# jujuC31/NeutFEM

Measured on AMD Instinct MI355X. Metric: outer power-iters/sec (IAEA-3D RT0-P0 k-eigenvalue solve), higher is better.
Workload: dtype f64; 1 GPU; IAEA-3D resampled 256x256x256 RT0-P0 2g, full Schur path, CG tol 0.0001, Chebyshev; cells=16777216, groups=2, parallelism=1 process(es) x 1 z-slab(s) each; RCCL: interface planes + scalar all-reduces

## Files before the change

neutfem_amd/csrc/neutfem_hip.hip:

```cpp
#include "../../include/neutfem_hip.h"
#include "nf_kernels.h"
#include "nf_assembly.h"
#include "nf_line_groups.h"
#include "nf_small_eig.h"

#include <dlfcn.h>
#include <unistd.h>

#include <algorithm>
#include <chrono>
#include <climits>
#include <cmath>
#include <cstdarg>
#include <cstdint>
#include <cstdio>
#include <cstdlib>
#include <cstring>
#include <map>
#include <mutex>
#include <string>
#include <type_traits>
#include <utility>
#include <vector>

// ... 42 lines not shown
};
static Rccl g_rccl;
static bool trace_comm() { static int on = -1; if (on < 0) { const char *e = getenv("NEUTFEM_TRACE_COMM"); on = e && atoi(e) ? 1 : 0; } return on == 1; }
#define TRACE_COMM(...) do { if (trace_comm()) { fprintf(stderr, "[comm] " __VA_ARGS__); fputc('\n', stderr); } } while (0)
static const int NCCL_DOUBLE = 8, NCCL_SUM = 0, NCCL_MAX = 2;
#define NCCLCHK(x) do { int r_ = (x); if (r_ != 0) return fail(NF_ERR_HIP, "%s failed: %s", #x, g_rccl.GetErrorString ? g_rccl.GetErrorString(r_) : "rccl error"); } while (0)

static int rccl_load()
{
    if (g_rccl.lib) return NF_OK;
    const char *env = getenv("NEUTFEM_RCCL_LIB");
    const char *names[] = { env ? env : "/opt/rocm/lib/librccl.so.1", "/opt/rocm/lib/librccl.so.1", "librccl.so.1", "librccl.so" };
    for (const char *n : names) { g_rccl.lib = dlopen(n, RTLD_NOW | RTLD_LOCAL); if (g_rccl.lib) break; }
    if (!g_rccl.lib) return fail(NF_ERR_HIP, "cannot load librccl.so: %s", dlerror());
#define SYM(field, name) do { *(void **)(&g_rccl.field) = dlsym(g_rccl.lib, name); if (!g_rccl.field) return fail(NF_ERR_HIP, "librccl.so lacks %s", name); } while (0)
    SYM(GetUniqueId, "ncclGetUniqueId"); SYM(CommInitRank, "ncclCommInitRank"); SYM(CommDestroy, "ncclCommDestroy");
    SYM(AllReduce, "ncclAllReduce"); SYM(Send, "ncclSend"); SYM(Recv, "ncclRecv"); SYM(GroupStart, "ncclGroupStart");
    SYM(GroupEnd, "ncclGroupEnd"); SYM(GetErrorString, "ncclGetErrorString");
#undef SYM
    *(void **)(&g_rccl.CommAbort) = dlsym(g_rccl.lib, "ncclCommAbort");
    *(void **)(&g_rccl.CommCount) = dlsym(g_rccl.lib, "ncclCommCount");
    Dl_info di;
    if (dladdr((void *)g_rccl.AllReduce, &di) && di.dli_fname) snprintf(g_rccl.path, sizeof g_rccl.path, "%s", di.dli_fname);
    return NF_OK;
}

struct nf_solver;
struct Transient;
struct nf_team {
    std::vector<nf_solver *> slabs;
    int device = 0;
    hipStream_t stream = nullptr;
    hipStream_t comm_stream = nullptr;
    hipStream_t y_stream = nullptr; hipEvent_t ev_fork = nullptr, ev_join = nullptr;
    int opt_xy_overlap = 1; long xy_overlap_max_cells = 6L << 20;
    hipEvent_t ev_z1 = nullptr, ev_xchg = nullptr;
    int nproc = 1, rank = 0;
    ncclComm_t comm = nullptr;
    ncclComm_t comm_x = nullptr; int opt_xchg_comm = 0;
    int opt_cg1 = -1, last_cg_reductions = 0; long cg1_max_cells = 1L << 40, team_max_cells = 0;
    int last_cg_form = 0;
    int opt_endpoint_w = 1, last_endpoint_w = 0;
    bool rccl_reduce = false;
    double *d_partials = nullptr; long partial_stride = 0, slab_cap = 0;
    CgScalars *d_cg = nullptr;
    double *d_out = nullptr;
    double *d_red = nullptr;
    double *d_errsrc = nullptr;
    double *d_vec = nullptr; long vec_stride = 0;
    int vec_cnt_pq = 0, vec_cnt_rr = 0; bool vec_ok = false; int opt_vec_reduce = 1, last_vec_reduce = 0;
    bool dead = false;
    bool poisoned = false; int poison_rc = 0; char poison_msg[256] = { 0 };
    int xchg_in_apply = 0;
    long cg_iter_total = 0;
    int inject_rank = -1; long inject_iter = -1;
    int inject_outer = -1; char inject_where = 0;
    double comm_timeout_s = 120.0;
    nf_progress_fn progress_fn = nullptr; void *progress_user = nullptr;
    volatile long outers_done = 0;
    bool linked_ready = false;
    int sep_sweeps = 0;
    std::vector<int> last_its;
    int last_outer = 0, coarse_outer = 0; long last_cg_total = 0;
    std::vector<double> hist_k, hist_dk, hist_dphi; std::vector<int> hist_cg;
    int has_valid_keff = 0; double last_keff = 1.0;
    HostPub *h_pub = nullptr, *d_pub = nullptr; unsigned long long pub_seq = 0; int opt_pub = 1;
    bool profile = false; long prof_tick = 0; int prof_every = 8;
    std::map<std::string, ProfSlot> prof;
    struct Ev { hipEvent_t a, b; int slot; };
    std::vector<Ev> ev_pending; std::vector<std::pair<hipEvent_t, hipEvent_t>> ev_free;
    int cg_batch = 0;
    int opt_nt_loads = 1; long nt_min_cells = 8000000;
    int opt_fuse = 1, opt_xcd = -1, opt_outer_dev = 1, opt_lean = 1, opt_lean_grid = RED_GRID, opt_sepfold = 1;
    long lean_max_cells = 4L << 20;
    OuterState *d_ost = nullptr; double *d_hist = nullptr; int hist_cap = 0;
    int opt_s_tx = 0, opt_s_seg = 0, opt_wsmin = 0;
    int opt_x_p2 = 0;
    int opt_split_dot = 1;
    int opt_s_long_dirs = 3;
    int s_long_min_y = 255;
    int opt_line_dict = -1, line_dict_dirs = 7, line_dict_fp_bits = 128; long line_dict_max_bytes = 512L * 1024;
    int opt_s_long = -1, s_long_min = 256;
    int opt_c_early = -1;
    size_t lds_limit = 160 * 1024;
    int opt_fuse3 = 1; long fuse3_max_cells = 400000;
    int opt_sens_grid = RED_GRID;
    int opt_cgx = 1, opt_keffx = 1, xcd_id = 0, xcd_groups = 32, last_xcd = 0; long xcd_min_cells = 2000, xcd_max_cells = 28000, xcd_solves = 0, xcd_refused = 0;
    XcdState *d_xcd = nullptr; double *d_xpart = nullptr;
    int opt_resident = 1, opt_resident_lds = 1, opt_resident_serial = 1, opt_resident_two_sided = 1, last_resident_serial = 0; long resident_max_dofs = 2500, resident_serial_max_dofs = 5120;
    int *d_hist_cg = nullptr; int hist_cg_cap = 0; ResidentOut *d_rout = nullptr;
    int last_path = 0;
    long direct_max_dofs = 6000;
    int last_direct = 0;
    long standin_unconverged = 0;
    std::vector<nf_solver *> cc; int cc_f[3] = {0, 0, 0};
};

struct nf_solver {
    int device = 0;
    nf_team *team = nullptr;
    int slab_index = 0;
    int if_lo = 0, if_hi = 0;
    int dim = 1, nx = 1, ny = 1, nz = 1, ng = 1, k = 0, m = 0;
    int n1 = 1, nloc = 1, nb = 0;
    long N = 0, nphi = 0, nJ = 0, nJx = 0, nJy = 0, nJz = 0;
    std::vector<double> xb, yb, zb, hx, hy, hz;
    double *d_hx = nullptr, *d_hy = nullptr, *d_hz = nullptr, *d_xb = nullptr, *d_yb = nullptr, *d_zb = nullptr;
    int bc_set[8] = {0}, bc_type[8] = {0};
    double *d_D = nullptr, *d_SigR = nullptr, *d_NSF = nullptr, *d_Chi = nullptr;
    std::vector<double *> d_SigS;
    bool xs_uploaded = false, built = false, diag_valid = false;
    unsigned char *d_void = nullptr; std::vector<unsigned char> void_host; double void_gamma = 0.0; long void_cells = 0;
    double *d_Cd = nullptr, *d_Mf = nullptr, *d_Mchi = nullptr;
    double *d_phi_adj = nullptr;
    double *d_modes[2] = {nullptr, nullptr}; int modes_n[2] = {0, 0}, modes_cap[2] = {0, 0};
    int has_valid_adjoint = 0; double last_keff_adj = 1.0;
    double *d_gamma = nullptr, *d_gpt_w = nullptr, *d_gpt_sc = nullptr; bool gpt_valid = false;
    std::vector<double *> d_Ms;
    const double **d_Ms_tab = nullptr;
    double *d_L[3] = {nullptr, nullptr, nullptr}, *d_DR[3] = {nullptr, nullptr, nullptr}, *d_D0[3] = {nullptr, nullptr, nullptr};
    long nlines[3] = {0, 0, 0};
    bool ld_tried = false, ld_use[3] = {false, false, false}; int ld_rejected = 0, ld_pitch[3] = {0, 0, 0};
    int *d_lid[3] = {nullptr, nullptr, nullptr}; double *d_ltab[3] = {nullptr, nullptr, nullptr};
    std::vector<long> ld_off[3]; std::vector<int> ld_rows[3]; size_t ld_bytes = 0;
    double *d_Sinv = nullptr;
    double *d_Sdense = nullptr; bool dense_valid = false;
    double *d_alo = nullptr, *d_ahi = nullptr, *d_hlo = nullptr, *d_hhi = nullptr, *d_gfl = nullptr;
    double *d_sinv_lo = nullptr, *d_sinv_hi = nullptr;
    double *d_clo = nullptr, *d_chi = nullptr, *d_rlo = nullptr, *d_rhi = nullptr, *d_ulo = nullptr, *d_uhi = nullptr;
    double *d_ctlo = nullptr, *d_cthi = nullptr, *d_elo = nullptr, *d_ehi = nullptr, *d_relo = nullptr, *d_rehi = nullptr;
    double *d_Wlo = nullptr, *d_Whi = nullptr; bool w_valid = false;
    double *d_phi = nullptr, *d_raw = nullptr;
    double *d_p0 = nullptr, *d_p1 = nullptr;
    double *d_tf = nullptr, *d_rhs = nullptr, *d_r = nullptr, *d_p = nullptr, *d_q = nullptr;
    double *d_p2 = nullptr, *d_qy = nullptr, *d_qz = nullptr;
    bool raw_valid = false, raw_is_diag = false;
    double *d_qsrc = nullptr;
    double src_total = 0.0; bool src_any = false;
    Transient *tr = nullptr; long build_gen = 0;
    long tr_rebuilds = 0;
    int opt_tr_rebalance = 1;
    double *d_Jz = nullptr; bool jz_valid = false;
    double *d_Jzb = nullptr;
    bool cmfd_init = false, cmfd_iface = false; double cmfd_relax = 1.0;
    double *d_Dt[3] = {nullptr, nullptr, nullptr}, *d_Dh[3] = {nullptr, nullptr, nullptr}; long nfc[3] = {0, 0, 0};
    double *d_cm = nullptr, *d_cmJ = nullptr; CmfdScalars *d_cmsc = nullptr;
    int cmfd_last_its = 0;
};

const char *nf_last_error(void) { return g_err.c_str(); }

static void coarse_cache_drop(nf_team *T)
{
    if (!T || T->cc.empty()) return;
    std::string keep = g_err;
    std::vector<nf_solver *> cc; cc.swap(T->cc);
    for (int i = (int)cc.size() - 1; i >= 0; --i) if (cc[i]) nf_destroy(cc[i]);
    g_err = keep;
}

int nf_device_count(void)
{
    int n = 0;
    if (hipGetDeviceCount(&n) != hipSuccess) { (void)hipGetLastError(); return 0; }
    return n;
}
// ... 121 lines not shown
    }
    if (const char *e = getenv("NEUTFEM_COMM_TIMEOUT_S")) { const double v = atof(e); if (v > 0) T->comm_timeout_s = v; }
    T->last_its.assign(64, 0);
    return NF_OK;
}
static void team_free(nf_team *T)
{
    if (!T) return;
    (void)hipSetDevice(T->device);
    if (T->dead) {
        delete T;
        return;
    }
    if (T->stream) (void)hipStreamSynchronize(T->stream);
    for (auto &e : T->ev_pending) { (void)hipEventDestroy(e.a); (void)hipEventDestroy(e.b); }
    for (auto &e : T->ev_free) { (void)hipEventDestroy(e.first); (void)hipEventDestroy(e.second); }
    if (T->comm_x && g_rccl.CommDestroy) g_rccl.CommDestroy(T->comm_x);
    if (T->comm && g_rccl.CommDestroy) g_rccl.CommDestroy(T->comm);
    if (T->d_xcd) (void)hipFree(T->d_xcd);
    dfree(T->d_xpart);
    dfree(T->d_partials); dfree(T->d_cg); dfree(T->d_out); dfree(T->d_red); dfree(T->d_errsrc); dfree(T->d_vec); dfree(T->d_ost); dfree(T->d_hist); dfree(T->d_hist_cg); dfree(T->d_rout);
    if (T->h_pub) (void)hipHostFree(T->h_pub);
    if (T->comm_stream) { (void)hipStreamSynchronize(T->comm_stream); (void)hipStreamDestroy(T->comm_stream); }
    if (T->y_stream) { (void)hipStreamSynchronize(T->y_stream); (void)hipStreamDestroy(T->y_stream); }
    if (T->ev_fork) (void)hipEventDestroy(T->ev_fork);
    if (T->ev_join) (void)hipEventDestroy(T->ev_join);
    if (T->ev_z1) (void)hipEventDestroy(T->ev_z1);
    if (T->ev_xchg) (void)hipEventDestroy(T->ev_xchg);
    if (T->stream) (void)hipStreamDestroy(T->stream);
    delete T;
}
static PartSegs segs_for(const nf_team *T, const std::vector<int> &counts)
{
    PartSegs ps; ps.n = (int)T->slabs.size();
    for (int i = 0; i < ps.n; ++i) { ps.off[i] = (int)(i * T->slab_cap); ps.cnt[i] = counts[i]; }
    return ps;
}

static int create_impl(int rt_order, int p_order, int ng, int nxb, const double *xb, int nyb, const double *yb, int nzb,
                       const double *zb, int if_lo, int if_hi, int device, nf_handle *out)
{
    if (!out || !xb || nxb < 2 || ng < 1 || ng > 64) return fail(NF_ERR_ARG, "nf_create: bad arguments");
    int k = std::min(rt_order, 2), m = std::min(p_order, 2);
    if (k < m) m = k;
    int ndev = nf_device_count();
    if (ndev <= 0) return fail(NF_ERR_NO_DEVICE, "nf_create: no HIP device visible (the gfx950 path has no CPU fallback)");
    if (device < 0 || device >= ndev) return fail(NF_ERR_ARG, "nf_create: device %d out of range (%d devices)", device, ndev);
    HIPCHK(hipSetDevice(device));
    nf_solver *S = new nf_solver();
    S->device = device; S->k = k; S->m = m; S->ng = ng; S->if_lo = if_lo; S->if_hi = if_hi;
    S->xb.assign(xb, xb + nxb);
    if (nyb > 1) S->yb.assign(yb, yb + nyb); else S->yb.assign(1, nyb == 1 && yb ? yb[0] : 0.0);
    if (nzb > 1) S->zb.assign(zb, zb + nzb); else S->zb.assign(1, nzb == 1 && zb ? zb[0] : 0.0);
    S->nx = nxb - 1; S->ny = nyb > 1 ? nyb - 1 : 1; S->nz = nzb > 1 ? nzb - 1 : 1;
    S->dim = S->nz > 1 ? 3 : (S->ny > 1 ? 2 : 1);
    if ((if_lo || if_hi) && (S->dim != 3 || S->nz < 3)) { delete S; return fail(NF_ERR_ARG, "a slab needs a 3D mesh with at least 3 z-planes"); }
    if (S->dim == 3 && (nyb < 2 || !yb)) { delete S; return fail(NF_ERR_ARG, "nf_create: a 3D mesh needs at least 2 y breaks (got %d)", nyb); }
    S->N = (long)S->nx * S->ny * S->nz;
    S->n1 = m + 1; S->nloc = 1; for (int t = 0; t < S->dim; ++t) S->nloc *= S->n1;
    S->nphi = S->N * S->nloc; S->nb = std::min(k, m);
    S->hx.resize(S->nx); S->hy.assign(S->ny, 1.0); S->hz.assign(S->nz, 1.0);
    for (int i = 0; i < S->nx; ++i) S->hx[i] = xb[i + 1] - xb[i];
    if (S->dim >= 2) for (int i = 0; i < S->ny; ++i) S->hy[i] = yb[i + 1] - yb[i];
    if (S->dim == 3) for (int i = 0; i < S->nz; ++i) S->hz[i] = zb[i + 1] - zb[i];
    for (auto *h : { &S->hx, &S->hy, &S->hz })
        for (double v : *h)
            if (!(v > 0.0) || !std::isfinite(v)) { delete S; return fail(NF_ERR_ARG, "nf_create: mesh breaks must be finite and strictly increasing (cell width %g)", v); }
    {
        int nf = 1, ni = k; for (int t = 1; t < S->dim; ++t) { nf *= k + 1; ni *= k + 1; }
        S->nJx = (long)(S->nx + 1) * S->ny * S->nz * nf;
        S->nJy = S->dim >= 2 ? (long)S->nx * (S->ny + 1) * S->nz * nf : 0;
        S->nJz = S->dim == 3 ? (long)S->nx * S->ny * (S->nz + 1) * nf : 0;
        S->nJ = S->nJx + S->nJy + S->nJz + S->N * S->dim * ni;
    }
    S->nlines[0] = (long)S->ny * S->nz; S->nlines[1] = (long)S->nx * S->nz; S->nlines[2] = (long)S->nx * S->ny;
    nf_team *T = new nf_team();
    T->device = device; T->slabs.push_back(S); S->team = T; S->slab_index = 0;
    {
        int a = 0, b = 0;
        if (hipDeviceGetAttribute(&a, hipDeviceAttributeMaxSharedMemoryPerBlock, device) != hipSuccess) a = 0;
        if (hipDeviceGetAttribute(&b, hipDeviceAttributeSharedMemPerBlockOptin, device) != hipSuccess) b = 0;
        (void)hipGetLastError();
        T->lds_limit = (size_t)std::max(std::max(a, b), 64 * 1024);
    }
    const char *cb = getenv("NEUTFEM_CG_BATCH"); T->cg_batch = cb ? atoi(cb) : 0;
    *out = S;
    int rc = NF_OK;
    if (const char *e = getenv("NEUTFEM_OPTS")) {
        std::string all(e); size_t pos = 0;
        while (pos < all.size()) {
            const size_t c = all.find(',', pos); const std::string kv = all.substr(pos, c == std::string::npos ? std::string::npos : c - pos);
            const size_t eq = kv.find('=');
            if (eq != std::string::npos && nf_set_option(S, kv.substr(0, eq).c_str(), atol(kv.c_str() + eq + 1)) != NF_OK) fprintf(stderr, "NEUTFEM_OPTS: %s\n", nf_last_error());
            if (c == std::string::npos) break;
            pos = c + 1;
        }
    }
    auto up = [&](double **d, const std::vector<double> &h) {
        if (rc != NF_OK) return;
        rc = dalloc(d, h.size());
        if (rc == NF_OK && hipMemcpy(*d, h.data(), h.size() * sizeof(double), hipMemcpyHostToDevice) != hipSuccess)
            rc = fail(NF_ERR_HIP, "nf_create: upload failed");
    };
    if (hipStreamCreateWithFlags(&T->stream, hipStreamNonBlocking) != hipSuccess) rc = fail(NF_ERR_HIP, "hipStreamCreate failed");
    if (rc == NF_OK && (if_lo || if_hi)) {
        if (hipStreamCreateWithFlags(&T->comm_stream, hipStreamNonBlocking) != hipSuccess || hipEventCreateWithFlags(&T->ev_z1, hipEventDisableTiming) != hipSuccess ||
            hipEventCreateWithFlags(&T->ev_xchg, hipEventDisableTiming) != hipSuccess ||
            hipStreamCreateWithFlags(&T->y_stream, hipStreamNonBlocking) != hipSuccess || hipEventCreateWithFlags(&T->ev_fork, hipEventDisableTiming) != hipSuccess ||
            hipEventCreateWithFlags(&T->ev_join, hipEventDisableTiming) != hipSuccess) rc = fail(NF_ERR_HIP, "comm stream / event creation failed");
    }
    up(&S->d_hx, S->hx); up(&S->d_hy, S->hy); up(&S->d_hz, S->hz); up(&S->d_xb, S->xb); up(&S->d_yb, S->yb); up(&S->d_zb, S->zb);
    const size_t NN = (size_t)S->nphi * ng;
    if (rc == NF_OK) rc = dalloc(&S->d_phi, NN);
    if (rc == NF_OK) rc = dalloc(&S->d_raw, NN);
    if (rc == NF_OK) rc = dalloc(&S->d_tf, S->nphi);
    if (rc == NF_OK) rc = dalloc(&S->d_rhs, S->nphi);
    if (rc == NF_OK) rc = dalloc(&S->d_r, S->nphi);
    if (rc == NF_OK) rc = dalloc(&S->d_p, S->nphi);
    if (rc == NF_OK) rc = dalloc(&S->d_q, S->nphi);
    if (rc == NF_OK && (if_lo || if_hi)) {
        const size_t nl = (size_t)S->nlines[2] * n_modes(S);
        double **arrs[] = { &S->d_clo, &S->d_chi, &S->d_rlo, &S->d_rhi, &S->d_ulo, &S->d_uhi, &S->d_ctlo, &S->d_cthi, &S->d_elo, &S->d_ehi, &S->d_relo, &S->d_rehi };
        for (auto a : arrs) if (rc == NF_OK) { rc = dalloc(a, nl); if (rc == NF_OK) (void)hipMemset(*a, 0, nl * sizeof(double)); }
    }
    if (rc == NF_OK) rc = team_alloc(T);
    if (rc != NF_OK) { nf_destroy(S); *out = nullptr; return rc; }
    S->d_SigS.assign((size_t)ng * ng, nullptr); S->d_Ms.assign((size_t)ng * ng, nullptr);
    return nf_reset_flux(S);
}

int nf_create(int rt_order, int p_order, int ng, int nxb, const double *xb, int nyb, const double *yb, int nzb,
              const double *zb, int device, nf_handle *out)
{
    return create_impl(rt_order, p_order, ng, nxb, xb, nyb, yb, nzb, zb, 0, 0, device, out);
}
int nf_create_slab(int rt_order, int p_order, int ng, int nxb, const double *xb, int nyb, const double *yb, int nzb,
                   const double *zb_slab, int interface_below, int interface_above, int device, nf_handle *out)
{
    return create_impl(rt_order, p_order, ng, nxb, xb, nyb, yb, nzb, zb_slab, interface_below ? 1 : 0, interface_above ? 1 : 0, device, out);
}

int nf_destroy(nf_handle S)
{
    if (!S) return NF_OK;
    (void)hipSetDevice(S->device);
    nf_team *T = S->team;
    if (T && T->dead) {
        std::vector<nf_solver *> cc; cc.swap(T->cc);
        for (auto *c : cc) if (c) nf_destroy(c);
        T->slabs.erase(std::remove(T->slabs.begin(), T->slabs.end(), S), T->slabs.end());
        if (T->slabs.empty()) team_free(T);
        delete S;
        return NF_OK;
    }
    coarse_cache_drop(T);
    transient_drop(S);
    if (T && T->stream) (void)hipStreamSynchronize(T->stream);
    for (int d = 0; d < 3; ++d) { dfree(S->d_Dt[d]); dfree(S->d_Dh[d]); }
    dfree(S->d_cm); dfree(S->d_cmJ); dfree(S->d_cmsc);
    dfree(S->d_hx); dfree(S->d_hy); dfree(S->d_hz); dfree(S->d_xb); dfree(S->d_yb); dfree(S->d_zb);
    dfree(S->d_D); dfree(S->d_SigR); dfree(S->d_NSF); dfree(S->d_Chi); dfree(S->d_void);
    for (auto &p : S->d_SigS) dfree(p);
    for (auto &p : S->d_Ms) dfree(p);
    dfree(S->d_Ms_tab);
    dfree(S->d_Cd); dfree(S->d_Mf); dfree(S->d_Mchi); dfree(S->d_phi_adj); dfree(S->d_Sinv); dfree(S->d_Sdense);
    for (int d = 0; d < 3; ++d) { dfree(S->d_L[d]); dfree(S->d_DR[d]); dfree(S->d_D0[d]); dfree(S->d_lid[d]); dfree(S->d_ltab[d]); }
// ... 653 lines not shown
template <unsigned N, class F> static bool with_index(unsigned key, F &&f) { return with_index(key, f, std::make_integer_sequence<unsigned, N>()); }

constexpr bool schur_x_legal(int NCH, bool VEC, int NB, bool NT, bool P2, bool DICT)
{
    return NCH >= 1 && NCH <= (NB == 0 ? 32 : 8) && (NCH & (NCH - 1)) == 0 && NB >= 0 && NB <= 2
        && (!NT || (VEC && NB == 0)) && (!P2 || (NT && NCH >= 2)) && (!DICT || (NT && NCH <= X_DICT_MAX_NCH));
}
struct XPlan { int lpl_log2 = 0, NCH = 0; unsigned grid = 0; bool vec = false, nt = false, p2 = false, xcd = false, dict = false; };
static XPlan x_plan(const nf_solver *S, bool fused = false)
{
    XPlan P; const int K = 2;
    const int lanes = (S->nx + K - 1) / K;
    while ((1 << P.lpl_log2) < lanes && P.lpl_log2 < 6) ++P.lpl_log2;
    const int LPL = 1 << P.lpl_log2, LPW = 64 / LPL;
    const int nch = (S->nx + LPL * K - 1) / (LPL * K);
    P.grid = (unsigned)((S->nlines[0] + 4 * LPW - 1) / (4 * LPW));
    for (int c = 1; c <= (S->nb == 0 ? 32 : 8); c *= 2) if (nch <= c) { P.NCH = c; break; }
    P.vec = S->nx % 2 == 0; P.nt = x_nt(S, S->nb);
    P.p2 = x_p2(S, S->nb, P.NCH, fused && x_fuses(S), P.nt); P.xcd = x_xcd(S, P.nt); P.dict = x_dict(S, S->nb, P.NCH, P.nt);
    return P;
}
static int launch_x(const nf_solver *S, int g, const ModeArgs &ma0, const Geom &G, int last, double *partials, const PassCg &P, int *nparts)
{
    const XPlan xp = x_plan(S, P.fuse.p != nullptr);
    if (!xp.NCH) return fail(NF_ERR_UNSUPPORTED, "nx = %d exceeds the x-line kernel limit (%d cells)", S->nx, S->nb == 0 ? 4096 : 1024);
    if (nparts) *nparts = (int)xp.grid * n_modes(S);
    const CgFuse fz = x_fuses(S) ? P.fuse : CgFuse{ nullptr, nullptr, nullptr };
    const ModeTab mt = mode_tab(S, 0);
    const dim3 gr(xp.grid, (unsigned)mt.n);
    const int first = 1 | (xp.xcd ? 2 : 0);
    const DictArgs da = dict_args(S, 0, g, xp.dict);
    ModeArgs ma = ma0; if (da.on) ma.Cd[0] = da.C;
    const double *L = da.on ? da.L : S->d_L[0] + g * S->N, *DR = da.on ? da.DR : S->d_DR[0] + g * S->N, *D0 = S->d_D0[0] + g * S->nlines[0];
    int lg = 0; while ((1 << lg) < xp.NCH) ++lg;
    const unsigned key = ((((unsigned)lg * 3 + (unsigned)S->nb) * 2 + xp.vec) * 2 + xp.nt) * 4 + xp.p2 * 2 + xp.dict;
    const bool hit = with_index<6 * 3 * 16>(key, [&](auto i) {
        constexpr unsigned I = decltype(i)::value;
        constexpr int NCH = 1 << (I / 48), NB = I / 16 % 3; constexpr bool VEC = I & 8, NT = I & 4, P2 = I & 2, DICT = I & 1;
        if constexpr (!schur_x_legal(NCH, VEC, NB, NT, P2, DICT)) return false;
        else hipLaunchKernelGGL((k_schur_x<2, NCH, VEC, NB, NT, P2, DICT>), gr, dim3(256), 0, S->team->stream, ma, mt, G, L, DR, D0, S->nx, S->ny, S->nlines[0], xp.lpl_log2,
                                first, last, partials, P.cg, fz, P.lean, da.ld);
        return true;
    });
    return hit ? NF_OK : fail(NF_ERR_ARG, "k_schur_x: no instantiation for NCH = %d, NB = %d, vec %d, nt %d, p2 %d, dict %d", xp.NCH, S->nb, xp.vec, xp.nt, xp.p2, xp.dict);
}

struct ChunkPlan { bool ok = false; int NS = 0, TX = 0; size_t lds = 0; };
static ChunkPlan chunk_plan(const nf_solver *S, int d)
{
    ChunkPlan P; const nf_team *T = S->team;
    const int n = d == 1 ? S->ny : S->nz;
    if (S->nb != 0 || d < 1 || d >= S->dim || (d == 2 && (S->if_lo || S->if_hi)) || !((T->opt_s_long_dirs >> (d - 1)) & 1)) return P;
    const int nmin = d == 1 ? T->s_long_min_y : T->s_long_min;
    if (!(T->opt_s_long == 1 || (T->opt_s_long < 0 && n > nmin)) || (size_t)S->N * sizeof(double) >= (1ull << 32)) return P;
    P.NS = (n + 15) / 16;
    P.TX = T->opt_s_tx ? T->opt_s_tx : 32;
    while (P.TX > 8 && P.TX * P.NS > 1024) P.TX >>= 1;
    while (P.TX > 8 && P.TX / 2 >= S->nx) P.TX >>= 1;
    P.lds = (size_t)(3 * P.TX * P.NS + 2 * P.TX + 16 + 2 * 8 * P.NS * P.TX) * sizeof(double);
    P.ok = P.TX * P.NS <= 1024 && P.lds <= T->lds_limit;
    if (P.ok && n <= 256 && T->opt_s_long < 1) {
        const long tiles = (long)((S->nx + P.TX - 1) / P.TX) * (d == 1 ? S->nz : S->ny);
        if (tiles < 1024) P.ok = false;
    }
    return P;
}

static dim3 c_grid(const nf_solver *S, int d, const ChunkPlan &cp) { return dim3((unsigned)((S->nx + cp.TX - 1) / cp.TX), (unsigned)(d == 1 ? S->nz : S->ny)); }
static unsigned c_block(const ChunkPlan &cp) { return (unsigned)((cp.TX * cp.NS + 63) / 64 * 64); }
static const int C_SEG = 8, C_NCH = 2;
static bool c_nt(const nf_solver *S) { return nt_regime(S); }
static bool c_dict(const nf_solver *S, int d, bool nt) { return nt && dict_dir(S, d); }
static const int C_EARLY_AUTO = 2;
static int c_early(const nf_solver *S, bool dict) { const int e = S->team->opt_c_early; return dict ? (e < 0 ? C_EARLY_AUTO : e) : 0; }
static int c_xcd(const nf_solver *S, int d, bool nt) { const nf_team *T = S->team; return T->opt_xcd >= 0 ? (T->opt_xcd >> (d - 1)) & 1 : (d == 1 && nt); }
static int s_xcd(const nf_solver *S, int d, int zmode)
{
    const nf_team *T = S->team;
    return T->opt_xcd >= 0 ? (T->opt_xcd >> (d - 1)) & 1 : ((d == 1 && nt_regime(S)) || ((zmode == 1 || zmode == 2) && S->N <= (6L << 20)));
}
static bool s_nt(const nf_solver *S, int zmode, int SEG) { return zmode != 3 && S->nb == 0 && SEG == 8 && nt_regime(S); }
static bool s_dict(const nf_solver *S, int d, int zmode, int SEG) { return zmode == 0 && s_nt(S, zmode, SEG) && dict_dir(S, d); }
static bool s_zw(const nf_solver *S, int zmode, bool zw_dot, bool want_dot) { return zmode == 0 && S->nb == 0 && zw_dot && want_dot; }
static bool s_fold(const nf_team *T, int zmode) { return zmode == 2 && T->sep_sweeps == 0 && T->opt_sepfold; }
static bool xcd_permutes(bool order, unsigned tiles) { return order && tiles % 8 == 0 && tiles > 8; }
static SegPlan seg_plan(const nf_solver *S, int d, int zmode)
{
    SegPlan P; const nf_team *T = S->team;
    const int n = d == 1 ? S->ny : S->nz, nouter = d == 1 ? S->nz : S->ny;
    P.SEG = T->opt_s_seg ? T->opt_s_seg : (S->nb > 0 ? ((n <= 256 || (S->nb == 2 && n <= 512)) ? 4 : 8) : (n <= 1024 ? 8 : (n <= 2048 ? 16 : 32)));
    P.NSEG = (n + P.SEG - 1) / P.SEG;
    if (P.NSEG > 128) { P.rc = fail(NF_ERR_UNSUPPORTED, "line length %d exceeds the segmented kernel limit", n); return P; }
    P.TX = T->opt_s_tx ? T->opt_s_tx : 64;
    const int tmax = zmode != 0 ? 512 : 1024;
    while (P.TX > 8 && P.TX * P.NSEG > tmax) P.TX >>= 1;
    if (P.TX * P.NSEG > tmax) { P.rc = fail(NF_ERR_UNSUPPORTED, "line length %d needs more than %d threads per block", n, tmax); return P; }
    while (P.TX > 8 && P.TX / 2 >= S->nx) P.TX >>= 1;
    P.grid = dim3((unsigned)((S->nx + P.TX - 1) / P.TX), (unsigned)nouter, (unsigned)n_modes(S)); P.block = dim3((unsigned)((P.TX * P.NSEG + 63) / 64 * 64));
    P.nparts = (int)(P.grid.x * P.grid.y * P.grid.z);
    P.lds = (size_t)(4 * P.TX * (P.NSEG + 1) + P.TX + 32) * sizeof(double);
    return P;
}
static const int LINE_DICT_AUTO_DIRS = 7;
static bool line_dict_eligible(const nf_solver *S, int d)
{
    const nf_team *T = S->team;
    if (T->opt_line_dict == 0 || d >= S->dim || T->slabs.size() != 1 || S->if_lo || S->if_hi || S->k != 0 || S->nb != 0 || S->nloc != 1 || !nt_regime(S)) return false;
    const int dirs = T->line_dict_dirs & (T->opt_line_dict < 0 ? LINE_DICT_AUTO_DIRS : 7);
    if (!((dirs >> d) & 1)) return false;
    if (d == 0) { const int nch = x_plan(S).NCH; return x_nt(S, 0) && nch >= 1 && nch <= X_DICT_MAX_NCH; }
    if (chunk_plan(S, d).ok && c_nt(S)) return true;
    const SegPlan sp = seg_plan(S, d, 0);
    return sp.rc == NF_OK && s_nt(S, 0, sp.SEG);
}
static int line_dict_prepare(nf_team *T)
{
    static_assert(sizeof(LineFp) == sizeof(nf_fp128), "fingerprints travel as they are");
    for (auto *S : T->slabs) {
        if (S->ld_tried || !S->built) continue;
        S->ld_tried = true;
        hipStream_t st = T->stream;
        const int ng = S->ng;
        for (int d = 0; d < S->dim; ++d) {
            if (!line_dict_eligible(S, d)) continue;
            const long nl = S->nlines[d], N = S->N;
            const int n = d == 0 ? S->nx : d == 1 ? S->ny : S->nz, pitch = (n + 15) / 16 * 16, narr = d == 0 ? 3 : 2;
            const unsigned gl = (unsigned)((nl + 63) / 64);
            auto Cd = [&](int g) { return d == 0 ? (const double *)(S->d_Cd + (size_t)g * S->nphi) : (const double *)nullptr; };
            DevTmp<LineFp> fp; NFCHK(dalloc(&fp.p, (size_t)nl * ng));
            for (int g = 0; g < ng; ++g)
                hipLaunchKernelGGL(k_line_fp, dim3(gl), dim3(64), 0, st, d, S->nx, S->ny, S->nz, (const double *)(S->d_L[d] + g * N), (const double *)(S->d_DR[d] + g * N),
                                   (const double *)(S->d_D0[d] + g * nl), Cd(g), nl, T->line_dict_fp_bits, fp.p + (size_t)g * nl);
            std::vector<nf_fp128> h((size_t)nl * ng);
            HIPCHK(hipMemcpyAsync(h.data(), fp.p, h.size() * sizeof(nf_fp128), hipMemcpyDeviceToHost, st));
            HIPCHK(hipStreamSynchronize(st));
            std::vector<int> ids((size_t)nl * ng), reps, rows(ng), idg, repg;
            std::vector<long> off(ng);
            bool fits = true; long total = 0;
            for (int g = 0; g < ng; ++g) {
                rows[g] = nf_group_lines(h.data() + (size_t)g * nl, nl, idg, repg);
                std::copy(idg.begin(), idg.end(), ids.begin() + (size_t)g * nl);
                reps.insert(reps.end(), repg.begin(), repg.end());
                off[g] = total; total += (long)rows[g] * pitch * narr;
                fits = fits && (long)rows[g] * 4 <= nl && (long)rows[g] * pitch * narr * (long)sizeof(double) <= T->line_dict_max_bytes;
            }
            if (!fits) continue;
            DevTmp<int> drep, dmis; int mism = 0;
            NFCHK(dalloc(&drep.p, reps.size())); NFCHK(dalloc(&dmis.p, 1));
            NFCHK(dalloc(&S->d_lid[d], ids.size())); NFCHK(dalloc(&S->d_ltab[d], (size_t)total));
            HIPCHK(hipMemcpyAsync(S->d_lid[d], ids.data(), ids.size() * sizeof(int), hipMemcpyHostToDevice, st));
            HIPCHK(hipMemcpyAsync(drep.p, reps.data(), reps.size() * sizeof(int), hipMemcpyHostToDevice, st));
            HIPCHK(hipMemsetAsync(dmis.p, 0, sizeof(int), st));
            long roff = 0;
            for (int g = 0; g < ng; ++g) {
                const double *L = S->d_L[d] + g * N, *DR = S->d_DR[d] + g * N;
                double *tL = S->d_ltab[d] + off[g], *tR = tL + (long)rows[g] * pitch, *tC = d == 0 ? tR + (long)rows[g] * pitch : nullptr;
                hipLaunchKernelGGL(k_line_verify, dim3(gl), dim3(64), 0, st, d, S->nx, S->ny, S->nz, L, DR, (const double *)(S->d_D0[d] + g * nl), Cd(g), nl,
                                   (const int *)(S->d_lid[d] + (size_t)g * nl), (const int *)(drep.p + roff), dmis.p);
                hipLaunchKernelGGL(k_line_gather, dim3((unsigned)(((long)rows[g] * pitch + 255) / 256)), dim3(256), 0, st, d, S->nx, S->ny, S->nz, L, DR, Cd(g),
                                   (const int *)(drep.p + roff), rows[g], pitch, tL, tR, tC);
                roff += rows[g];
            }
            HIPCHK(hipMemcpyAsync(&mism, dmis.p, sizeof(int), hipMemcpyDeviceToHost, st));
            HIPCHK(hipStreamSynchronize(st));
            HIPCHK(hipGetLastError());
            if (mism) { S->ld_rejected |= 1 << d; dfree(S->d_lid[d]); dfree(S->d_ltab[d]); continue; }
            S->ld_use[d] = true; S->ld_pitch[d] = pitch; S->ld_off[d] = off; S->ld_rows[d] = rows;
            S->ld_bytes += (size_t)total * sizeof(double) + ids.size() * sizeof(int);
        }
    }
    return NF_OK;
}
struct SPass { int rc = NF_OK; bool chunked = false; ChunkPlan cp; SegPlan seg; unsigned V = 0; int xcd = 0, early = 0; bool fold = false, fuse = false; };
static std::string variant_name(unsigned V)
{
    static const char *const bit[] = { "fuse", "nt", "zw", "sr", "dict" };
    std::string r;
    for (int i = 0; i < 5; ++i) if (V >> i & 1) r += (r.empty() ? "" : "+") + std::string(bit[i]);
    return r;
}
static SPass s_pass(const nf_solver *S, int d, int zmode, bool want_dot, bool zw_dot, bool fuse, bool cg1, bool chunks = true)
{
    SPass R;
    if (chunks && zmode == 0) R.cp = chunk_plan(S, d);
    if (R.cp.ok && (!want_dot || zw_dot)) {
        const bool nt = c_nt(S), dict = c_dict(S, d, nt);
        R.chunked = true; R.V = (nt ? SV_NT : 0) | (want_dot ? SV_ZW : 0) | (dict ? SV_DICT : 0);
        R.xcd = c_xcd(S, d, nt); R.early = c_early(S, dict);
        return R;
    }
    R.seg = seg_plan(S, d, zmode);
    if ((R.rc = R.seg.rc) != NF_OK) return R;
    const int SEG = R.seg.SEG; const bool p0 = S->nb == 0;
    R.fuse = fuse && zmode == 1 && S->nloc == 1;
    const bool sr = cg1 && p0 && SEG == 8 && d == 2 && ((zmode == 1 && R.fuse) || (zmode == 2 && want_dot));
    R.V = (R.fuse && p0 ? SV_FUSE : 0) | (s_nt(S, zmode, SEG) ? SV_NT : 0) | (s_zw(S, zmode, zw_dot, want_dot) ? SV_ZW : 0)
        | (sr ? SV_SR : 0) | (s_dict(S, d, zmode, SEG) ? SV_DICT : 0);
    R.xcd = s_xcd(S, d, zmode); R.fold = s_fold(S->team, zmode);
    return R;
}
static int launch_s(const nf_solver *S, int d, int g, const ModeArgs &ma, const Geom &G, int last, double *partials, const PassCg &P, int *nparts, int zmode)
{
    const nf_team *T = S->team; const CgScalars *cg = P.cg;
    const long N = S->N;
    const int n = d == 1 ? S->ny : S->nz;
    const long nxy = (long)S->nx * S->ny;
    const long sl = d == 1 ? S->nx : nxy, ostride = d == 1 ? nxy : S->nx;
    const double *L = S->d_L[d] + g * N, *DR = S->d_DR[d] + g * N, *D0 = S->d_D0[d] + g * S->nlines[d];
    auto pick = [&](bool chunks) { return s_pass(S, d, zmode, last && partials, P.zw_dot, P.fuse.p != nullptr, P.cg1.red != nullptr, chunks); };
    SPass ps = pick(true);
    if (ps.chunked) {
        const ChunkPlan &cp = ps.cp;
        const dim3 grid = c_grid(S, d, cp), block(c_block(cp));
        const DictArgs da = dict_args(S, d, g, (ps.V & SV_DICT) != 0);
        const unsigned key = ((unsigned)ps.early * 2 + da.on) * 4 + ((ps.V & SV_NT) ? 2 : 0) + (unsigned)(d - 1);
        bool launched = false;
        const bool hit = with_index<3 * 2 * 2 * 2>(key, [&](auto i) {
            constexpr unsigned I = decltype(i)::value;
            constexpr int DIR = 1 + (I & 1), EARLY = I / 8; constexpr bool NT = I & 2, DICT = I & 4;
            if constexpr (!schur_c_legal(DIR, NT, DICT, EARLY)) return false;
            else if (lds_opt_in((const void *)k_schur_c<DIR, NT, DICT, EARLY>, cp.lds)) {
                hipLaunchKernelGGL((k_schur_c<DIR, NT, DICT, EARLY>), grid, block, cp.lds, T->stream, ma.x[0], ma.y[0], ma.Ta, da.on ? da.L : L, da.on ? da.DR : DR, D0, n, sl, ostride,
                                   S->nx, cp.TX, cp.NS, last, partials, cg, ps.xcd, da.ld);
                launched = hipGetLastError() == hipSuccess;
            }
            return true;
        });
        if (!hit) return fail(NF_ERR_ARG, "k_schur_c: no instantiation for direction %d, nt %d, dict %d, early %d", d, (ps.V & SV_NT) ? 1 : 0, da.on ? 1 : 0, ps.early);
        if (launched) { if (nparts) *nparts = (int)(grid.x * grid.y); return NF_OK; }
        ps = pick(false);
    }
    if (ps.rc != NF_OK) return ps.rc;
    const ModeTab mt = mode_tab(S, d);
    if (nparts) *nparts = ps.seg.nparts;
    hipStream_t st = P.stream ? P.stream : T->stream;
    SlabArgs sa; memset(&sa, 0, sizeof sa);
    sa.noacc = P.noacc ? 1 : 0; sa.yadd = P.yadd;
    sa.xcd = ps.xcd;
    sa.wsmin = T->opt_wsmin;
    const CgFuse fz = ps.fuse ? P.fuse : CgFuse{ nullptr, nullptr, nullptr };
    const CgLean lz = fz.p ? P.lean_z1 : CgLean{ nullptr, nullptr, 0, 0, 0 };
    if (ps.V & SV_SR) {
        sa.sr = P.cg1; sa.sr_r = S->d_r; sa.sr_q = S->d_q; sa.sr_stride = T->partial_stride;
        sa.sr_part = T->d_partials + 3 * T->partial_stride + (long)S->slab_index * T->slab_cap;
    }
    const DictArgs da = dict_args(S, d, g, (ps.V & SV_DICT) != 0);
    if (zmode != 0) {
        const long nl = S->nlines[2];
        sa.if_lo = S->if_lo; sa.if_hi = S->if_hi; sa.mode = zmode;
        sa.alo = S->d_alo + g * nl; sa.ahi = S->d_ahi + g * nl; sa.ulo = S->d_ulo; sa.uhi = S->d_uhi; sa.clo = S->d_clo; sa.chi = S->d_chi;
        if (zmode == 3) {
            int nfa = 1, ni = S->k; for (int t = 1; t < S->dim; ++t) { nfa *= S->k + 1; ni *= S->k + 1; }
            sa.nfa = nfa; sa.ni = ni;
            sa.jz = S->d_Jz + (size_t)g * S->nJz; sa.jzb = S->d_Jzb ? S->d_Jzb + (size_t)g * S->N * ni : nullptr;
            for (int m = 0; m < mt.n && m < 9; ++m) {
                int amode = 0, q = m, mul = 1;
                for (int t = 0; t < S->dim; ++t) { if (t == d) continue; amode += (q % S->n1) * mul; q /= S->n1; mul *= S->k + 1; }
                sa.amode[m] = amode;
            }
        }
        if (ps.fold) {
            sa.fold = 1; sa.rlo = S->d_rlo; sa.rhi = S->d_rhi; sa.sinv_lo = S->d_sinv_lo + g * nl; sa.sinv_hi = S->d_sinv_hi + g * nl;
        }
    }
    int lg = 0; while ((4 << lg) < ps.seg.SEG) ++lg;
    const unsigned key = (4 << lg) == ps.seg.SEG ? ((ps.V * 3 + (zmode != 0 ? 2u : d - 1u)) * 3 + (unsigned)S->nb) * 4 + (unsigned)lg : ~0u;
    const bool hit = with_index<(SV_ALL + 1) * 3 * 3 * 4>(key, [&](auto i) {
        constexpr unsigned I = decltype(i)::value, V = I / 36;
        constexpr int SEG = 4 << (I & 3), NB = I / 4 % 3, DIR = I / 12 % 3 == 0 ? 1 : 2; constexpr bool SLAB = I / 12 % 3 == 2;
        if constexpr (!schur_s_legal(SEG, DIR, SLAB, NB, V)) return false;
        else hipLaunchKernelGGL((k_schur_s<SEG, DIR, SLAB, NB, V>), ps.seg.grid, ps.seg.block, ps.seg.lds, st, ma, mt, G, da.on ? da.L : L, da.on ? da.DR : DR, D0, n, sl, ostride, S->nx,
                                ps.seg.TX, ps.seg.NSEG, last, partials, cg, sa, fz, lz, da.ld);
        return true;
    });
    return hit ? NF_OK : fail(NF_ERR_ARG, "k_schur_s: no instantiation for SEG = %d (s_seg), direction %d, zmode %d, NB = %d, variant \"%s\"", ps.seg.SEG, d, zmode, S->nb, variant_name(ps.V).c_str());
}

static dim3 endpoint_w_grid(const nf_solver *S) { return dim3((unsigned)((S->nx + 63) / 64), (unsigned)S->ny); }
static bool endpoint_w_taken(const nf_team *T, const nf_solver *S, bool sr, bool fuse_reads_x)
{
    const dim3 gr = endpoint_w_grid(S);
    return sr && S->w_valid && T->opt_endpoint_w && fuse_reads_x && (long)gr.x * gr.y <= T->slab_cap;
}
static int team_endpoint_phase(nf_team *T, int g, const std::vector<const double *> &xs, const std::vector<double *> &ys, const ApplyCg &A,
                               hipEvent_t after_z1, bool need_u = false, std::vector<int> *cnt3 = nullptr)
{
    const int ns = (int)T->slabs.size(); const CgScalars *cg = A.cg;
    for (int i = 0; i < ns; ++i) {
        const nf_solver *S = T->slabs[i];
        if (cnt3) (*cnt3)[i] = 0;
        if (!(S->if_lo || S->if_hi)) continue;
        const PassCg P = pass_cg(A, S, i);
        if (endpoint_w_taken(T, S, P.cg1.red != nullptr, P.fuse.p == xs[i])) {
            const dim3 gr = endpoint_w_grid(S);
            {
                hipLaunchKernelGGL(k_endpoint_w, gr, dim3(256), 0, T->stream, P.fuse.p, const_cast<double *>(P.fuse.r), (const double *)S->d_q, P.fuse.xsol,
                                   (const double *)(S->d_Wlo + (size_t)g * S->N), (const double *)(S->d_Whi + (size_t)g * S->N), S->d_clo, S->d_chi,
                                   S->nx, S->ny, S->nz, S->if_lo, S->if_hi, 40, P.cg1, cg, T->d_partials + 3 * T->partial_stride + (long)S->slab_index * T->slab_cap);
                if (cnt3) (*cnt3)[i] = (int)(gr.x * gr.y);
                T->last_endpoint_w = 1;
                continue;
            }
        }
        NFCHK(launch_s(S, 2, g, mode_args(S, g, 2, 0, xs[i], ys[i]), make_geom(S), 0, nullptr, P, nullptr, 1));
    }
    if (after_z1) (void)hipEventRecord(after_z1, T->stream);
    HIPCHK(hipEventRecord(T->ev_z1, T->stream));
    HIPCHK(hipStreamWaitEvent(T->comm_stream, T->ev_z1, 0));
    NFCHK(exchange_planes(T, 0, 0, T->comm_stream));
    auto each_slab = [&](auto &&launch) {
        for (int i = 0; i < ns; ++i) {
            nf_solver *S = T->slabs[i];
            if (S->if_lo || S->if_hi) launch(S, S->nlines[2], dim3((unsigned)((S->nlines[2] * n_modes(S) + 255) / 256)));
        }
    };
    if (need_u || !s_fold(T, 2))
        each_slab([&](nf_solver *S, long nl, dim3 gr) {
            hipLaunchKernelGGL(k_separators, gr, dim3(256), 0, T->comm_stream, S->d_clo, S->d_chi, S->d_rlo, S->d_rhi, S->d_sinv_lo + g * nl, S->d_sinv_hi + g * nl,
                               S->d_ulo, S->d_uhi, S->d_ctlo, S->d_cthi, nl, nl * n_modes(S), S->if_lo, S->if_hi, cg); });
    for (int sweep = 0; sweep < T->sep_sweeps; ++sweep) {
        each_slab([&](nf_solver *S, long nl, dim3 gr) {
            hipLaunchKernelGGL(k_sep_couple, gr, dim3(256), 0, T->comm_stream, S->d_gfl + g * nl, S->d_ulo, S->d_uhi, S->d_elo, S->d_ehi, nl, nl * n_modes(S), S->if_lo, S->if_hi, cg); });
        NFCHK(exchange_planes(T, 2, 0, T->comm_stream));
        each_slab([&](nf_solver *S, long nl, dim3 gr) {
            hipLaunchKernelGGL(k_sep_update, gr, dim3(256), 0, T->comm_stream, S->d_ctlo, S->d_cthi, S->d_elo, S->d_ehi, S->d_relo, S->d_rehi,
                               S->d_sinv_lo + g * nl, S->d_sinv_hi + g * nl, S->d_ulo, S->d_uhi, nl, nl * n_modes(S), S->if_lo, S->if_hi, cg); });
    }
    HIPCHK(hipEventRecord(T->ev_xchg, T->comm_stream));
    return NF_OK;
}

static bool team_is_single(const nf_team *T) { return T->slabs.size() == 1 && !T->slabs[0]->if_lo && !T->slabs[0]->if_hi; }
static bool split_dot(const nf_team *T, bool want_dot, bool lean)
{
    const int dim = T->slabs[0]->dim;
    bool split = want_dot && dim >= 2 && team_is_single(T) && T->slabs[0]->nb == 0 && !lean && T->opt_split_dot;
    if (split && T->opt_split_dot < 2) split = chunk_plan(T->slabs[0], dim - 1).ok;
    return split;
}
static bool xy_overlap(const nf_team *T, bool any_if, bool prof)
{
    const bool xy = T->slabs[0]->dim == 3 && any_if && T->opt_xy_overlap && T->slabs[0]->nb == 0 && T->y_stream && !prof;
    bool xy_all = xy; if (xy) for (auto *X : T->slabs) xy_all = xy_all && X->N <= T->xy_overlap_max_cells && !chunk_plan(X, 1).ok;
    return xy_all;
}

static int team_schur_apply(nf_team *T, int g, const std::vector<const double *> &xs, const std::vector<double *> &ys, bool want_dot,
                            const ApplyCg &A, std::vector<int> *counts = nullptr, std::vector<int> *cnt3 = nullptr)
{
    const int ns = (int)T->slabs.size();
    const int dim = T->slabs[0]->dim;
    bool any_if = false; for (auto *S : T->slabs) any_if |= S->if_lo || S->if_hi;
    hipEvent_t a, b, ta = nullptr, tb = nullptr;
    const bool prof = T->profile && (T->prof_tick++ % T->prof_every == 0);
    if (prof) prof_begin(T, 3, &ta, &tb);
    if (any_if) {
        if (prof) prof_begin(T, 4, &a, &b);
        NFCHK(team_endpoint_phase(T, g, xs, ys, A, prof ? b : nullptr, false, cnt3));
// ... 164 lines not shown
    }
    A.nx = S->nx; A.ny = S->ny; A.dim = S->dim; A.nlines_x = S->nlines[0]; A.N = S->nphi;
    A.nmodes = n_modes(S);
    for (int d = 0; d < 3; ++d) A.mt[d] = mode_tab(S, d < S->dim ? d : 0);
    int lanes = (S->nx + 1) / 2, lpl_log2 = 0;
    while ((1 << lpl_log2) < lanes && lpl_log2 < 5) ++lpl_log2;
    int nch = (lanes + (1 << lpl_log2) - 1) >> lpl_log2;
    if (nch == 1 && lpl_log2 == 5) {
        const int Pn = T->xcd_groups, tasks = (int)((S->nlines[0] + 1) / 2) * A.nmodes;
        int waves = (tasks + Pn - 1) / Pn;
        for (int r = 0; r < 2; ++r) if (S->dim >= r + 2) waves += (((P.A.gx[r] * P.A.gy[r] * A.nmodes + Pn - 1) / Pn) * P.A.TX[r] * P.A.NSEG[r] + 63) / 64;
        if (waves > XCD_THREADS / 64) { lpl_log2 = 4; nch = 2; }
    }
    if (nch > 2) return fail(NF_ERR_STATE, "k_cg_xcd: x lines of %d cells", S->nx);
    A.lpl_log2 = lpl_log2; A.ntask_x = (int)((S->nlines[0] + (64 >> lpl_log2) - 1) / (64 >> lpl_log2));
    for (int r = 0; r < 2; ++r) { A.n[r] = P.A.n[r]; A.TX[r] = P.A.TX[r]; A.NSEG[r] = P.A.NSEG[r]; A.gx[r] = P.A.gx[r]; A.gy[r] = P.A.gy[r]; A.sl[r] = P.A.sl[r]; A.ostride[r] = P.A.ostride[r]; }
    if (S->dim < 2) { A.TX[0] = A.NSEG[0] = 1; } if (S->dim < 3) { A.TX[1] = A.NSEG[1] = 1; }
    A.pA = S->d_p; A.pB = S->d_p2; A.r = S->d_r;
    A.part = T->d_xpart; A.st = T->d_xcd; A.xcc = T->xcd_id;
    *nch_out = nch;
    return NF_OK;
}
constexpr bool xcd_legal(int NCH, int NB, int SEG) { return NCH >= 1 && NCH <= 2 && NB >= 0 && NB <= 2 && SEG == (NB == 0 ? 8 : 4); }
template <int NCH_, bool VEC_, int NB_, int SEG_> struct XcdInst { static constexpr int NCH = NCH_, NB = NB_, SEG = SEG_; static constexpr bool VEC = VEC_; };
template <class F> static int xcd_select(const char *name, const nf_solver *S, const Fuse3Plan &P, int nch, F &&launch)
{
    int rc = NF_OK;
    const unsigned key = (P.seg == 4 || P.seg == 8) ? ((((unsigned)(nch - 1) * 2 + (P.vec ? 1u : 0u)) * 3 + (unsigned)S->nb) * 2 + (P.seg == 8 ? 1u : 0u)) : ~0u;
    const bool hit = with_index<2 * 2 * 3 * 2>(key, [&](auto i) {
        constexpr unsigned I = decltype(i)::value;
        constexpr int NCH = 1 + I / 12, NB = I / 2 % 3, SEG = (I & 1) ? 8 : 4; constexpr bool VEC = I / 6 % 2;
        if constexpr (!xcd_legal(NCH, NB, SEG)) return false;
        else { rc = launch(XcdInst<NCH, VEC, NB, SEG>()); return true; }
    });
    return hit ? rc : fail(NF_ERR_ARG, "%s: no instantiation for NCH = %d, vec %d, NB = %d, SEG = %d", name, nch, P.vec, S->nb, P.seg);
}
static const size_t XCD_LDS = (size_t)(5 * 1024 + 64 + 32) * sizeof(double);
static int launch_cg_xcd(nf_solver *S, int g, const Fuse3Plan &P, double *xsol, unsigned long long seq)
{
    nf_team *T = S->team; hipStream_t st = T->stream;
    XcdArgs A; int nch = 1;
    NFCHK(xcd_fill(S, g, P, A, &nch));
    A.xsol = xsol; A.cg = T->d_cg; A.hp = T->d_pub; A.seq = seq;
    const size_t lds = XCD_LDS; const unsigned G = 8u * (unsigned)T->xcd_groups;
    NFCHK(xcd_select("k_cg_xcd", S, P, nch, [&](auto t) -> int { using I = decltype(t);
        if (!lds_opt_in((const void *)k_cg_xcd<I::NCH, I::VEC, I::NB, I::SEG>, lds)) return fail(NF_ERR_HIP, "k_cg_xcd: %zu bytes of LDS refused", lds);
        hipLaunchKernelGGL((k_cg_xcd<I::NCH, I::VEC, I::NB, I::SEG>), dim3(G), dim3(XCD_THREADS), lds, st, A);
        return NF_OK;
    }));
    HIPCHK(hipGetLastError());
    return NF_OK;
}
enum CgForm { CG_XCD, CG_FUSE3, CG_LEAN, CG_FUSED, CG_CLASSIC, CG_TEAM_LEAN, CG_TEAM_VEC, CG_TEAM_SR };
static const char *const CG_FORM_NAME[] = { "xcd", "fuse3", "lean", "fused", "classic", "team_lean", "team_vec", "team_sr" };
struct CgPlan {
    CgForm form = CG_CLASSIC; Fuse3Plan f3; int gru = 0;
    bool fused = false; int reductions = 0;
    bool lean() const { return form == CG_XCD || form == CG_FUSE3 || form == CG_LEAN; }
};
static CgPlan cg_plan(const nf_team *T)
{
    CgPlan P; const nf_solver *S0 = T->slabs[0]; const bool single = team_is_single(T);
    P.fused = T->opt_fuse != 0 && (single || S0->nloc == 1);
    P.reductions = single ? 0 : 2;
    P.form = P.fused ? CG_FUSED : CG_CLASSIC;
    if (!P.fused || !T->opt_lean) return P;
    if (!single) {
        bool sr = T->opt_cg1 > 0 || (T->opt_cg1 < 0 && T->team_max_cells <= T->cg1_max_cells);
        for (auto *S : T->slabs) sr = sr && S->dim == 3 && S->nb == 0 && (T->opt_s_seg == 0 || T->opt_s_seg == 8) && S->nz <= 1024;
        const bool vec = T->nproc > 1 && T->slabs.size() == 1 && T->vec_ok && T->opt_vec_reduce;
        P.form = sr ? CG_TEAM_SR : vec ? CG_TEAM_VEC : CG_TEAM_LEAN; P.reductions = sr ? 1 : 2;
        return P;
    }
    if (T->rccl_reduce || S0->N > T->lean_max_cells) return P;
    P.form = CG_LEAN;
    P.gru = grid_for(S0->nphi, 256, T->opt_lean_grid);
    if (!T->opt_fuse3 || S0->N > T->fuse3_max_cells) return P;
    P.f3 = fuse3_plan(S0);
    if (P.f3.ok && P.f3.nblocks > T->slab_cap) P.f3.ok = false;
    if (P.f3.ok) P.form = xcd_eligible(T, S0, P.f3) ? CG_XCD : CG_FUSE3;
    return P;
}

struct PlanPass { const char *dir, *family; int mode, SEG, NCH, TX, NSEG; dim3 grid; unsigned block; bool nt, p2, zw, order; unsigned tiles; bool fold = false, dict = false; int early = 0; unsigned V = 0; };
static void plan_emit(std::string &js, const PlanPass &p)
{
    char tmp[416];
    snprintf(tmp, sizeof tmp, "%s{\"dir\": \"%s\", \"mode\": %d, \"family\": \"%s\", \"SEG\": %d, \"NCH\": %d, \"TX\": %d, \"NSEG\": %d, \"grid\": [%u, %u, %u], "
             "\"block\": %u, \"nt\": %d, \"p2\": %d, \"zw\": %d, \"xcd_order\": %d, \"xcd_permutes\": %d, \"fold\": %d, \"dict\": %d, \"early\": %d", js.back() == '[' ? "" : ", ", p.dir, p.mode, p.family,
             p.SEG, p.NCH, p.TX, p.NSEG, p.grid.x, p.grid.y, p.grid.z, p.block, p.nt ? 1 : 0, p.p2 ? 1 : 0, p.zw ? 1 : 0, p.order ? 1 : 0, xcd_permutes(p.order, p.tiles) ? 1 : 0, p.fold ? 1 : 0, p.dict ? 1 : 0, p.early);
    js += tmp;
    if (!strcmp(p.family, "s")) js += ", \"variant\": \"" + variant_name(p.V) + "\"";
    js += "}";
}
static int plan_s(std::string &js, const nf_solver *S, int d, int zmode, bool want_dot, bool zw_dot, bool fuse, bool cg1)
{
    const SPass ps = s_pass(S, d, zmode, want_dot, zw_dot, fuse, cg1);
    if (ps.rc != NF_OK) return ps.rc;
    const dim3 gr = ps.chunked ? c_grid(S, d, ps.cp) : ps.seg.grid;
    plan_emit(js, { d == 1 ? "y" : "z", ps.chunked ? "c" : "s", zmode, ps.chunked ? C_SEG : ps.seg.SEG, ps.chunked ? C_NCH : 1, ps.chunked ? ps.cp.TX : ps.seg.TX, ps.chunked ? ps.cp.NS : ps.seg.NSEG,
                    gr, ps.chunked ? c_block(ps.cp) : ps.seg.block.x, (ps.V & SV_NT) != 0, false, (ps.V & SV_ZW) != 0, ps.xcd != 0, gr.x * gr.y, ps.fold, (ps.V & SV_DICT) != 0, ps.early, ps.V });
    return NF_OK;
}
int nf_apply_plan(nf_handle S, int in_cg, char *json_buf, size_t len)
{
    if (!S || !json_buf || len < 2) return fail(NF_ERR_ARG, "nf_apply_plan: bad arguments");
    if (!S->built) return fail(NF_ERR_STATE, "nf_apply_plan: call nf_build first");
    HIPCHK(hipSetDevice(S->team->device));
    NFCHK(line_dict_prepare(S->team));
    const nf_team *T = S->team;
    const bool slab = S->if_lo || S->if_hi;
    if (!team_is_single(T) && !T->linked_ready) return fail(NF_ERR_STATE, "nf_apply_plan: run a team apply or solve first (the team has not been prepared since its options changed)");
    const CgPlan cp = cg_plan(T);
    const bool cg = in_cg != 0, fused = cg && cp.fused, lean = cg && cp.lean(), sr = cg && cp.form == CG_TEAM_SR;
    const bool split = split_dot(T, cg, lean);
    bool any_if = false; for (auto *X : T->slabs) any_if |= X->if_lo || X->if_hi;
    const bool xy_all = xy_overlap(T, any_if, false);
    char tmp[288];
    snprintf(tmp, sizeof tmp, "{\"in_cg\": %d, \"form\": \"%s\", \"slab\": %d, \"fused\": %d, \"lean\": %d, \"single_reduce\": %d, \"split_dot\": %d, \"xy_overlap\": %d, \"passes\": [",
             cg ? 1 : 0, cg ? CG_FORM_NAME[cp.form] : "", slab ? 1 : 0, fused ? 1 : 0, lean ? 1 : 0, sr ? 1 : 0, split ? 1 : 0, xy_all ? 1 : 0);
    std::string js = tmp;
    for (int d = 0; d < S->dim; ++d) {
        const bool last = d == S->dim - 1, want_dot = cg && (last || split);
        if (d == 0) {
            const XPlan xp = x_plan(S, fused);
            if (!xp.NCH) return fail(NF_ERR_UNSUPPORTED, "nx = %d exceeds the x-line kernel limit (%d cells)", S->nx, S->nb == 0 ? 4096 : 1024);
            plan_emit(js, { "x", "x", 0, 0, xp.NCH, 1 << xp.lpl_log2, 0, dim3(xp.grid, (unsigned)n_modes(S)), 256u, xp.nt, xp.p2, false, xp.xcd, xp.grid, false, xp.dict });
        } else if (d == 2 && slab) {
            if (endpoint_w_taken(T, S, sr, fused)) { const dim3 gr = endpoint_w_grid(S); plan_emit(js, { "z", "endpoint_w", 1, 0, 0, 64, 0, gr, 256u, false, false, false, false, gr.x * gr.y }); }
            else NFCHK(plan_s(js, S, 2, 1, false, false, fused, sr));
            NFCHK(plan_s(js, S, 2, 2, want_dot, split, fused, sr));
        } else if (d == 1 && xy_all) NFCHK(plan_s(js, S, 1, 0, false, split, fused, sr));
        else NFCHK(plan_s(js, S, d, 0, want_dot, split, fused, sr));
    }
    {
        int nd[3] = { 0, 0, 0 };
        for (int d = 0; d < S->dim; ++d) if (dict_dir(S, d)) nd[d] = *std::max_element(S->ld_rows[d].begin(), S->ld_rows[d].end());
        snprintf(tmp, sizeof tmp, "], \"line_dict\": {\"x\": %d, \"y\": %d, \"z\": %d}}", nd[0], nd[1], nd[2]);
        js += tmp;
    }
    if (js.size() + 1 > len) return fail(NF_ERR_ARG, "nf_apply_plan: buffer of %zu bytes is too small (%zu needed)", len, js.size() + 1);
    memcpy(json_buf, js.c_str(), js.size() + 1);
    return NF_OK;
}

struct CgRun {
    nf_team *T; int g; const CgPlan &P; CgForm form; const std::vector<double *> &x;
    std::vector<const double *> ps; std::vector<double *> qs;
    std::vector<int> gcnt, acnt, cnt3;
    bool any_if = false;
    double *row1() const { return T->d_partials + T->partial_stride; }
    double *vec_rr() const { return T->d_vec + T->vec_stride; }
    int chk(int rc) const { return team_poison(T, rc, form == CG_TEAM_VEC) ? rc : NF_OK; }
    template <class F> void each_slab(F &&launch) const { if (!T->poisoned) for (size_t i = 0; i < T->slabs.size(); ++i) launch(T->slabs[i], (int)i); }
};
static ApplyCg cg_apply_args(const CgRun &R, int index)
{
    nf_team *T = R.T; const int first = index == 0 ? 1 : 0;
    ApplyCg A; A.cg = T->d_cg; A.fused = R.P.fused; A.xsol = &R.x;
    if (R.form == CG_FUSE3 || R.form == CG_LEAN) A.lean = CgLean{ T->d_cg, R.row1(), R.P.gru, index & 1, first };
    if (R.form == CG_TEAM_SR) A.cg1 = Cg1{ T->d_red, T->d_cg, index };
    if (R.form == CG_TEAM_VEC) A.lean_z1 = CgLean{ T->d_cg, R.vec_rr(), T->vec_cnt_rr, index & 1, first, T->vec_cnt_rr };
    if (R.form == CG_TEAM_LEAN) A.lean_z1 = CgLean{ T->d_cg, T->d_red + 2, -1, index & 1, first };
    return A;
}
static int cg_step_fuse3(CgRun &R, int index)
{
    nf_team *T = R.T; nf_solver *S0 = T->slabs[0];
    double *A = S0->d_p, *B = S0->d_p2;
    double *pin = (index == 0 || (index & 1)) ? A : B, *pout = pin == A ? B : A;
    hipEvent_t ta = nullptr, tb = nullptr;
    const bool prof = T->profile && (T->prof_tick++ % T->prof_every == 0);
    if (prof) prof_begin(T, 3, &ta, &tb);
    const int rc = launch_apply3(S0, R.g, R.P.f3, pin, pout, R.x[0], cg_apply_args(R, index).lean);
    if (prof) (void)hipEventRecord(tb, T->stream);
    with_void(S0, [&](auto M, VoidMask vm) {
        hipLaunchKernelGGL(k_cg_rupdate3<decltype(M)::value>, dim3(R.P.gru), dim3(256), 0, T->stream, S0->d_r, (const double *)S0->d_q, (const double *)(S0->dim >= 2 ? S0->d_qy : nullptr),
                           (const double *)(S0->dim == 3 ? S0->d_qz : nullptr), S0->nphi, T->d_cg, R.row1(), CgLean{ T->d_cg, T->d_partials, R.P.f3.nblocks, index & 1, 0 }, vm); });
    return rc;
}
static int cg_step_apply(CgRun &R, int index, long global_it)
{
    nf_team *T = R.T;
    T->xchg_in_apply = 0;
// ... 341 lines not shown
    hipStream_t st = S->team->stream;
    const long N = S->N, nJ = S->nJ;
    if (!S->raw_valid) { memset(J_host, 0, sizeof(double) * nJ * S->ng); return NF_OK; }
    const bool slab = S->if_lo || S->if_hi;
    if (slab) {
        if (S->raw_is_diag) NFCHK(team_reconstruct_Jz_diag(S->team));
        else NFCHK(team_reconstruct_Jz(S->team));
    }
    DevTmp<double> dJ_; NFCHK(dalloc(&dJ_.p, (size_t)nJ)); double *dJ = dJ_.p;
    int ni = S->k; for (int t = 1; t < S->dim; ++t) ni *= S->k + 1;
    const long nJface = S->nJx + S->nJy + S->nJz;
    const long foff[3] = { 0, S->nJx, S->nJx + S->nJy };
    for (int g = 0; g < S->ng; ++g) {
        NFCHK(flux_to_J(S, g, S->d_raw + (size_t)g * S->nphi, dJ, slab ? 2 : S->dim, S->raw_is_diag ? 1 : 0, st));
        if (slab) {
            HIPCHK(hipMemcpyAsync(dJ + foff[2], S->d_Jz + (size_t)g * S->nJz, S->nJz * sizeof(double), hipMemcpyDeviceToDevice, st));
            if (ni > 0 && !S->raw_is_diag && S->d_Jzb)
                HIPCHK(hipMemcpyAsync(dJ + nJface + 2L * N * ni, S->d_Jzb + (size_t)g * N * ni, (size_t)N * ni * sizeof(double), hipMemcpyDeviceToDevice, st));
        }
        HIPCHK(hipMemcpyAsync(J_host + (size_t)g * nJ, dJ, nJ * sizeof(double), hipMemcpyDeviceToHost, st));
        HIPCHK(hipStreamSynchronize(st));
    }
    HIPCHK(hipGetLastError());
    return NF_OK;
}

static const int CHEB_NMAX = 15;
static const double CHEB_SIGMA = 0.98;
static void cheb_tables(double *ca, double *cbv)
{
    const double sigma = CHEB_SIGMA, Gm = std::acosh(2. / sigma - 1.);
    ca[0] = cbv[0] = 0.; ca[1] = 2. / (2. - sigma); cbv[1] = 0.;
    for (int i = 2; i < CHEB_NMAX; ++i) { ca[i] = std::cosh((i - 1) * Gm) / std::cosh(i * Gm); cbv[i] = std::cosh((i - 2) * Gm) / std::cosh(i * Gm); }
}

static int dense_prepare(nf_team *T)
{
    nf_solver *S = T->slabs[0];
    if (S->dense_valid) return NF_OK;
    const int n = (int)S->nphi, ng = S->ng; const size_t nn = (size_t)n * n;
    hipStream_t st = T->stream;
    NFCHK(dalloc(&S->d_Sdense, nn * ng));
    DevTmp<double> work; NFCHK(dalloc(&work.p, nn));
    for (int g = 0; g < ng; ++g) {
        double *M = S->d_Sdense + (size_t)g * nn;
        for (int j = 0; j < n; ++j) {
            hipLaunchKernelGGL(k_unit_vector, dim3(grid_for(n)), dim3(256), 0, st, S->d_p, (long)n, (long)j);
            NFCHK(team_schur_apply(T, g, { S->d_p }, { M + (size_t)j * n }, false, ApplyCg()));
        }
        double *a = M, *b = work.p;
        const unsigned gr = (unsigned)((nn + 255) / 256);
        for (int k = 0; k < n; ++k) { hipLaunchKernelGGL(k_gj_step, dim3(gr), dim3(256), 0, st, (const double *)a, b, n, k); std::swap(a, b); }
        if (a != M) HIPCHK(hipMemcpyAsync(M, a, nn * sizeof(double), hipMemcpyDeviceToDevice, st));
        HIPCHK(hipStreamSynchronize(st));
    }
    HIPCHK(hipGetLastError());
    S->dense_valid = true;
    return NF_OK;
}
static void dense_solve(nf_team *T, int g, const double *rhs, double *sol)
{
    nf_solver *S = T->slabs[0];
    const int n = (int)S->nphi;
    hipLaunchKernelGGL(k_dense_matvec, dim3((unsigned)((n + 255) / 256)), dim3(256), 0, T->stream, (const double *)(S->d_Sdense + (size_t)g * n * n), rhs, sol, n);
}

static void team_copy_options(nf_team *C, const nf_team *T, bool same_mesh_kind)
{
    C->opt_cg1 = T->opt_cg1; C->cg1_max_cells = T->cg1_max_cells; C->opt_endpoint_w = T->opt_endpoint_w; C->opt_fuse = T->opt_fuse; C->opt_lean = T->opt_lean;
    C->opt_sepfold = T->opt_sepfold; C->opt_lean_grid = T->opt_lean_grid; C->lean_max_cells = T->lean_max_cells;
    C->opt_fuse3 = T->opt_fuse3; C->fuse3_max_cells = T->fuse3_max_cells; C->opt_cgx = T->opt_cgx; C->opt_keffx = T->opt_keffx;
    C->xcd_min_cells = T->xcd_min_cells; C->xcd_max_cells = T->xcd_max_cells; C->xcd_id = T->xcd_id; C->xcd_groups = T->xcd_groups;
    C->opt_resident = T->opt_resident; C->opt_resident_lds = T->opt_resident_lds; C->opt_resident_serial = T->opt_resident_serial;
    C->opt_resident_two_sided = T->opt_resident_two_sided; C->resident_max_dofs = T->resident_max_dofs; C->resident_serial_max_dofs = T->resident_serial_max_dofs;
    C->cg_batch = T->cg_batch; C->opt_outer_dev = T->opt_outer_dev; C->direct_max_dofs = T->direct_max_dofs;
    if (!same_mesh_kind) return;
    const bool dict_moved = C->opt_line_dict != T->opt_line_dict || C->line_dict_dirs != T->line_dict_dirs || C->line_dict_fp_bits != T->line_dict_fp_bits ||
                            C->line_dict_max_bytes != T->line_dict_max_bytes;
    const bool regime_moved = C->opt_nt_loads != T->opt_nt_loads || C->nt_min_cells != T->nt_min_cells || C->opt_s_long != T->opt_s_long || C->opt_s_long_dirs != T->opt_s_long_dirs ||
                              C->s_long_min != T->s_long_min || C->s_long_min_y != T->s_long_min_y || C->opt_s_seg != T->opt_s_seg || C->opt_s_tx != T->opt_s_tx;
    C->opt_line_dict = T->opt_line_dict; C->line_dict_dirs = T->line_dict_dirs; C->line_dict_fp_bits = T->line_dict_fp_bits; C->line_dict_max_bytes = T->line_dict_max_bytes;
    C->opt_nt_loads = T->opt_nt_loads; C->nt_min_cells = T->nt_min_cells; C->opt_s_long = T->opt_s_long; C->opt_s_long_dirs = T->opt_s_long_dirs;
    C->s_long_min = T->s_long_min; C->s_long_min_y = T->s_long_min_y; C->opt_s_seg = T->opt_s_seg; C->opt_s_tx = T->opt_s_tx;
    C->opt_wsmin = T->opt_wsmin; C->opt_c_early = T->opt_c_early; C->opt_x_p2 = T->opt_x_p2; C->opt_split_dot = T->opt_split_dot; C->opt_xcd = T->opt_xcd;
    C->opt_xy_overlap = T->opt_xy_overlap; C->xy_overlap_max_cells = T->xy_overlap_max_cells; C->opt_vec_reduce = T->opt_vec_reduce;
    C->opt_pub = T->opt_pub; C->opt_sens_grid = T->opt_sens_grid; C->prof_every = T->prof_every;
    if (dict_moved) { (void)hipSetDevice(C->device); for (auto *X : C->slabs) line_dict_drop(X); }
    else if (regime_moved) for (auto *X : C->slabs) if (!X->d_lid[0] && !X->d_lid[1] && !X->d_lid[2]) X->ld_tried = false;
}

static int solve_keff_impl(nf_team *T, const nf_keff_opts *o, double *keff, int *n_outer);

static int coarsen_slab(nf_solver *S, int rx, int ry, int rz, nf_handle *out)
{
    const int dim = S->dim, ng = S->ng;
    hipStream_t st = S->team->stream;
    const int nxc = S->nx / rx, nyc = S->ny / ry, nzc = S->nz / rz;
    std::vector<double> xc(nxc + 1), yc(dim >= 2 ? nyc + 1 : 1), zc(dim >= 3 ? nzc + 1 : 1);
    for (int a = 0; a <= nxc; ++a) xc[a] = S->xb[a * rx];
    if (dim >= 2) for (int j = 0; j <= nyc; ++j) yc[j] = S->yb[j * ry]; else yc[0] = 0.0;
    if (dim >= 3) for (int kk = 0; kk <= nzc; ++kk) zc[kk] = S->zb[kk * rz]; else zc[0] = 0.0;
    nf_handle C = nullptr;
    NFCHK(create_impl(0, 0, ng, nxc + 1, xc.data(), (int)yc.size(), yc.data(), (int)zc.size(), zc.data(), S->if_lo, S->if_hi, S->device, &C));
    *out = C;
    for (int a = 0; a < 8; ++a) if (S->bc_set[a]) nf_set_bc(C, a, S->bc_type[a]);
    const long Nc = C->N;
    auto coarsen = [&](const double *fine, double **coarse, int nfields) -> int {
        NFCHK(dalloc(coarse, (size_t)Nc * nfields));
        hipLaunchKernelGGL(k_coarsen, dim3((unsigned)((Nc + 127) / 128)), dim3(128), 0, st, fine, *coarse, S->d_xb, S->d_yb, S->d_zb,
                           dim, S->nx, S->ny, S->nz, rx, ry, rz, nfields);
        return NF_OK;
    };
    NFCHK(coarsen(S->d_D, &C->d_D, ng)); NFCHK(coarsen(S->d_SigR, &C->d_SigR, ng));
    NFCHK(coarsen(S->d_NSF, &C->d_NSF, ng)); NFCHK(coarsen(S->d_Chi, &C->d_Chi, ng));
    for (int b = 0; b < ng * ng; ++b)
        if (S->d_SigS[b]) NFCHK(coarsen(S->d_SigS[b], &C->d_SigS[b], 1));
    HIPCHK(hipStreamSynchronize(st));
    C->xs_uploaded = true;
    return nf_build(C);
}

static int coarse_init(nf_team *T, const nf_keff_opts *o, double *k_coarse, const std::vector<double *> &dsts, bool *done)
{
    *done = false;
    const int ns = (int)T->slabs.size();
    nf_solver *S0 = T->slabs[0];
    const int dim = S0->dim, ng = S0->ng;
    const int nf = o->n_coarse_factors;
    int rx = nf > 0 ? std::max(o->coarse_factors[0], 1) : 1;
    int ry = (nf > 1 && dim >= 2) ? std::max(o->coarse_factors[1], 1) : 1;
    int rz = (nf > 2 && dim >= 3) ? std::max(o->coarse_factors[2], 1) : 1;
    double bad = 0.0; const nf_solver *Sbad = nullptr;
    for (auto *S : T->slabs)
        if (S->nx % rx || S->ny % ry || S->nz % rz) { bad = 1.0; Sbad = S; }
    if (T->rccl_reduce && T->nproc > 1) {
        HIPCHK(hipMemcpyAsync(T->d_red, &bad, sizeof(double), hipMemcpyHostToDevice, T->stream));
        NCCLCHK(g_rccl.AllReduce(T->d_red, T->d_red, 1, NCCL_DOUBLE, NCCL_MAX, T->comm, T->stream));
        HIPCHK(hipMemcpyAsync(&bad, T->d_red, sizeof(double), hipMemcpyDeviceToHost, T->stream));
        NFCHK(team_stream_wait(T, T->stream));
    }
    if (bad != 0.0) {
        if (ns == 1 && T->nproc == 1) return NF_OK;
        if (Sbad) return fail(NF_ERR_ARG, "coarse factors (%d,%d,%d) do not divide slab %d x %d x %d", rx, ry, rz, Sbad->nx, Sbad->ny, Sbad->nz);
        return fail(NF_ERR_ARG, "coarse factors (%d,%d,%d) do not divide a slab on another rank", rx, ry, rz);
    }
    std::vector<nf_handle> C(ns, nullptr);
    int rc = NF_OK;
    const bool reuse = (int)T->cc.size() == ns && T->cc_f[0] == rx && T->cc_f[1] == ry && T->cc_f[2] == rz;
    if (reuse) {
        for (int i = 0; i < ns && rc == NF_OK; ++i) { C[i] = T->cc[i]; rc = nf_reset_flux(C[i]); }
    } else {
        coarse_cache_drop(T);
        for (int i = 0; i < ns && rc == NF_OK; ++i) rc = coarsen_slab(T->slabs[i], rx, ry, rz, &C[i]);
        if (rc == NF_OK && ns > 1) rc = nf_link_slabs(C.data(), ns);
        if (rc == NF_OK) { T->cc = C; T->cc_f[0] = rx; T->cc_f[1] = ry; T->cc_f[2] = rz; }
        else { std::string keep = g_err; for (int i = ns - 1; i >= 0; --i) if (C[i]) nf_destroy(C[i]); g_err = keep; return rc; }
    }
    nf_team *CT = rc == NF_OK ? C[0]->team : nullptr;
    if (CT) {
        CT->comm = T->comm; CT->nproc = T->nproc; CT->rank = T->rank; CT->rccl_reduce = T->rccl_reduce; CT->linked_ready = false;
        CT->comm_x = T->comm_x; team_copy_options(CT, T, false);
    }
    double kc = 1.0; int nout = 0;
    if (rc == NF_OK) {
        nf_keff_opts co = *o;
        co.tol_keff = o->tol_keff * 10.0; co.tol_flux = o->tol_flux * 10.0; co.max_outer = o->max_outer / 2;
        co.use_coarse_init = 0; co.n_coarse_factors = 0; co.use_diagonal_solver = 0; co.solver_type_pushed = 1; co.profile = 0; co.use_cmfd = 0;
// ... 2343 lines not shown
        (void)hipEventDestroy(a); (void)hipEventDestroy(b);
    }
    if (rc == NF_OK && (hipMemcpy(A_host, dA.p, (size_t)n_elems * nJ * nJ * sizeof(double), hipMemcpyDeviceToHost) != hipSuccess ||
                        hipMemcpy(B_host, dB.p, (size_t)n_elems * nP * nJ * sizeof(double), hipMemcpyDeviceToHost) != hipSuccess ||
                        hipMemcpy(C_host, dC.p, (size_t)n_elems * nP * nP * sizeof(double), hipMemcpyDeviceToHost) != hipSuccess))
        rc = fail(NF_ERR_HIP, "nf_local_matrices: download failed");
    return rc;
}

int nf_time_device_copy(nf_handle S, size_t bytes, int reps, double *gbps)
{
    if (!S || bytes < 16 || reps < 1 || !gbps) return fail(NF_ERR_ARG, "nf_time_device_copy: bad arguments");
    HIPCHK(hipSetDevice(S->device));
    hipStream_t st = S->team->stream;
    const long n2 = (long)(bytes / 16);
    nf_d2 *a = nullptr, *b = nullptr;
    NFCHK(dalloc(&a, (size_t)n2)); if (dalloc(&b, (size_t)n2) != NF_OK) { dfree(a); return NF_ERR_HIP; }
    (void)hipMemsetAsync(a, 0, (size_t)n2 * 16, st);
    hipEvent_t e0, e1; (void)hipEventCreate(&e0); (void)hipEventCreate(&e1);
    double best = 0.0; hipError_t e = hipSuccess;
    int ncu = 256; (void)hipDeviceGetAttribute(&ncu, hipDeviceAttributeMultiprocessorCount, S->device);
    const bool verbose = getenv("NEUTFEM_COPY_VERBOSE") != nullptr;
    struct V { int kind, per_cu; };
    const V vs[] = { {0, 16}, {0, 64}, {0, 256}, {0, 0}, {1, 16}, {1, 64}, {1, 256}, {1, 0}, {2, 64}, {2, 0}, {3, 0} };
    const int NV = (int)(sizeof vs / sizeof vs[0]);
    for (int variant = 0; variant < NV && e == hipSuccess; ++variant) {
        const V v = vs[variant];
        const int U = v.kind == 2 ? 8 : 4;
        const long full = (n2 + 256L * U - 1) / (256L * U);
        const int grid = (int)std::min<long>(v.per_cu ? (long)ncu * v.per_cu : full, full);
        auto once = [&]() {
            if (v.kind == 3) { (void)hipMemcpyAsync(b, a, (size_t)n2 * 16, hipMemcpyDeviceToDevice, st); return; }
            if (v.kind == 0) hipLaunchKernelGGL((k_copy<false, 4>), dim3(grid), dim3(256), 0, st, (const nf_d2 *)a, b, n2);
            else if (v.kind == 1) hipLaunchKernelGGL((k_copy<true, 4>), dim3(grid), dim3(256), 0, st, (const nf_d2 *)a, b, n2);
            else hipLaunchKernelGGL((k_copy<true, 8>), dim3(grid), dim3(256), 0, st, (const nf_d2 *)a, b, n2);
        };
        once();
        (void)hipEventRecord(e0, st);
        for (int i = 0; i < reps; ++i) once();
        (void)hipEventRecord(e1, st);
        e = hipEventSynchronize(e1);
        float ms = 0.f; (void)hipEventElapsedTime(&ms, e0, e1);
        const double gb = ms > 0.f ? 2.0 * (double)n2 * 16.0 * reps / (ms * 1e-3) / 1e9 : 0.0;
        if (verbose) fprintf(stderr, "[copy] variant %2d (%s, grid %d): %.0f GB/s\n", variant,
                             v.kind == 3 ? "hipMemcpyDtoD" : v.kind == 0 ? "plain, 4 in flight" : v.kind == 1 ? "nt, 4 in flight" : "nt, 8 in flight", v.kind == 3 ? 0 : grid, gb);
        if (e == hipSuccess) best = std::max(best, gb);
    }
    (void)hipEventDestroy(e0); (void)hipEventDestroy(e1);
    dfree(a); dfree(b);
    if (e != hipSuccess) return fail(NF_ERR_HIP, "nf_time_device_copy: %s", hipGetErrorString(e));
    *gbps = best;
    return NF_OK;
}

int nf_set_option(nf_handle S, const char *key, long value)
{
    if (!S || !key) return fail(NF_ERR_ARG, "nf_set_option: bad arguments");
    nf_team *T = S->team;
    if (!strcmp(key, "s_tx")) {
        if (value != 0 && value != 8 && value != 16 && value != 32 && value != 64) return fail(NF_ERR_ARG, "nf_set_option: s_tx must be 0 (auto), 8, 16, 32 or 64");
        T->opt_s_tx = (int)value;
        if (T->nproc > 1) T->linked_ready = false;
    } else if (!strcmp(key, "s_seg")) {
        if (value != 0 && value != 4 && value != 8 && value != 16 && value != 32) return fail(NF_ERR_ARG, "nf_set_option: s_seg must be 0 (auto), 4, 8, 16 or 32");
        T->opt_s_seg = (int)value;
        if (T->nproc > 1) T->linked_ready = false;
    }
    else if (!strcmp(key, "s_pair")) {  }
    else if (!strcmp(key, "s_wsmin")) T->opt_wsmin = (int)std::max(0L, std::min(100000L, value));
    else if (!strcmp(key, "vec_reduce")) T->opt_vec_reduce = value != 0;
    else if (!strcmp(key, "cg_single_reduce")) { T->opt_cg1 = value < 0 ? -1 : (value != 0); T->linked_ready = false; }
    else if (!strcmp(key, "cg_single_reduce_max_cells")) { T->cg1_max_cells = std::max(0L, value); T->linked_ready = false; }
    else if (!strcmp(key, "endpoint_weights")) { T->opt_endpoint_w = value != 0; T->linked_ready = false; }
    else if (!strcmp(key, "xchg_comm")) { T->opt_xchg_comm = value != 0; if (T->nproc > 1) T->linked_ready = false; }
    else if (!strcmp(key, "xy_overlap")) T->opt_xy_overlap = value != 0;
    else if (!strcmp(key, "xy_overlap_max_cells")) T->xy_overlap_max_cells = std::max(0L, value);
    else if (!strcmp(key, "split_dot")) T->opt_split_dot = (int)std::max(0L, std::min(2L, value));
    else if (!strcmp(key, "x_two_phase")) T->opt_x_p2 = value < 0 ? -1 : (value > 0 ? 1 : 0);
    else if (!strcmp(key, "s_long")) T->opt_s_long = value < 0 ? -1 : (value > 0 ? 1 : 0);
    else if (!strcmp(key, "s_long_dirs")) T->opt_s_long_dirs = (int)(value & 3);
    else if (!strcmp(key, "s_long_min_y")) T->s_long_min_y = (int)std::max(1L, std::min(1000000L, value));
    else if (!strcmp(key, "s_long_min")) T->s_long_min = (int)std::max(1L, std::min(1000000L, value));
    else if (!strcmp(key, "c_early")) T->opt_c_early = value < 0 ? -1 : (int)std::min(2L, value);
    else if (!strcmp(key, "line_dict") || !strcmp(key, "line_dict_dirs") || !strcmp(key, "line_dict_max_bytes") || !strcmp(key, "line_dict_fp_bits")) {
        if (!strcmp(key, "line_dict")) T->opt_line_dict = value < 0 ? -1 : (value > 0 ? 1 : 0);
        else if (!strcmp(key, "line_dict_dirs")) T->line_dict_dirs = (int)(value & 7);
        else if (!strcmp(key, "line_dict_max_bytes")) T->line_dict_max_bytes = std::max(0L, std::min(1L << 30, value));
        else T->line_dict_fp_bits = (int)std::max(0L, std::min(128L, value));
        HIPCHK(hipSetDevice(T->device));
        for (auto *X : T->slabs) line_dict_drop(X);
    }
    else if (!strcmp(key, "cg_batch")) T->cg_batch = (int)value;
    else if (!strcmp(key, "cg_fuse")) T->opt_fuse = value != 0;
    else if (!strcmp(key, "xcd")) T->opt_xcd = value < 0 ? -1 : (int)(value & 7);
    else if (!strcmp(key, "host_pub")) T->opt_pub = value != 0;
    else if (!strcmp(key, "prof_every")) { if (value < 1) return fail(NF_ERR_ARG, "prof_every must be >= 1"); T->prof_every = (int)value; }
    else if (!strcmp(key, "nt_loads")) T->opt_nt_loads = value != 0;
    else if (!strcmp(key, "nt_min_cells")) T->nt_min_cells = value;
    else if (!strcmp(key, "outer_dev")) T->opt_outer_dev = value != 0;
    else if (!strcmp(key, "cg_lean")) T->opt_lean = value != 0;
    else if (!strcmp(key, "sep_fold")) T->opt_sepfold = value != 0;
    else if (!strcmp(key, "cg_lean_max_cells")) T->lean_max_cells = value;
    else if (!strcmp(key, "resident")) T->opt_resident = value != 0;
    else if (!strcmp(key, "resident_lds")) T->opt_resident_lds = value != 0;
    else if (!strcmp(key, "resident_serial")) T->opt_resident_serial = value != 0;
    else if (!strcmp(key, "resident_two_sided")) T->opt_resident_two_sided = value != 0;
    else if (!strcmp(key, "resident_max_dofs")) { T->resident_max_dofs = value; T->resident_serial_max_dofs = std::min<long>(value, 5120); }
    else if (!strcmp(key, "resident_serial_max_dofs")) T->resident_serial_max_dofs = value;
    else if (!strcmp(key, "direct_max_dofs")) T->direct_max_dofs = std::max(0L, std::min(8192L, value));
    else if (!strcmp(key, "cg_fuse3")) T->opt_fuse3 = value != 0;
    else if (!strcmp(key, "cg_xcd")) T->opt_cgx = value != 0;
    else if (!strcmp(key, "keff_xcd")) T->opt_keffx = value != 0;
    else if (!strcmp(key, "cg_xcd_min_cells")) T->xcd_min_cells = value;
    else if (!strcmp(key, "cg_xcd_max_cells")) T->xcd_max_cells = value;
    else if (!strcmp(key, "cg_xcd_id")) T->xcd_id = (int)(value & 15);
    else if (!strcmp(key, "cg_xcd_groups")) T->xcd_groups = (int)std::max<long>(1, std::min<long>(value, 64));
    else if (!strcmp(key, "cg_fuse3_max_cells")) T->fuse3_max_cells = value;
    else if (!strcmp(key, "cg_lean_grid")) T->opt_lean_grid = (int)std::max(1L, std::min(1024L, value));
    else if (!strcmp(key, "sens_grid")) T->opt_sens_grid = (int)std::max(1L, std::min(65536L, value));
    else if (!strcmp(key, "transient_rebalance")) S->opt_tr_rebalance = value != 0;
    else return fail(NF_ERR_ARG, "nf_set_option: unknown key %s", key);
    if (!strcmp(key, "nt_loads") || !strcmp(key, "nt_min_cells") || !strncmp(key, "s_long", 6) || !strcmp(key, "s_seg") || !strcmp(key, "s_tx"))
        for (auto *X : T->slabs) if (!X->d_lid[0] && !X->d_lid[1] && !X->d_lid[2]) X->ld_tried = false;
    return NF_OK;
}

int nf_mem_info(int device, size_t *free_bytes, size_t *total_bytes)
{
    if (hipSetDevice(device) != hipSuccess) { (void)hipGetLastError(); return fail(NF_ERR_ARG, "nf_mem_info: device %d out of range", device); }
    size_t f = 0, t = 0;
    HIPCHK(hipMemGetInfo(&f, &t));
    if (free_bytes) *free_bytes = f;
    if (total_bytes) *total_bytes = t;
    return NF_OK;
}
int nf_dev_alloc(nf_handle S, size_t bytes, void **p)
{
    if (!S || !p) return fail(NF_ERR_ARG, "nf_dev_alloc: bad arguments");
    HIPCHK(hipSetDevice(S->device)); HIPCHK(hipMalloc(p, std::max<size_t>(bytes, 8))); return NF_OK;
}
int nf_dev_free(nf_handle S, void *p) { if (!S) return fail(NF_ERR_ARG, "null handle"); HIPCHK(hipSetDevice(S->device)); if (p) HIPCHK(hipFree(p)); return NF_OK; }
int nf_memcpy_h2d(nf_handle S, void *dst, const void *src, size_t bytes)
{
    if (!S || !dst || !src) return fail(NF_ERR_ARG, "nf_memcpy_h2d: bad arguments");
    HIPCHK(hipSetDevice(S->device)); HIPCHK(hipMemcpy(dst, src, bytes, hipMemcpyHostToDevice)); return NF_OK;
}
int nf_memcpy_d2h(nf_handle S, void *dst, const void *src, size_t bytes)
{
    if (!S || !dst || !src) return fail(NF_ERR_ARG, "nf_memcpy_d2h: bad arguments");
    HIPCHK(hipSetDevice(S->device)); HIPCHK(hipStreamSynchronize(S->team->stream)); HIPCHK(hipMemcpy(dst, src, bytes, hipMemcpyDeviceToHost)); return NF_OK;
}
int nf_synchronize(nf_handle S) { if (!S) return fail(NF_ERR_ARG, "null handle"); HIPCHK(hipSetDevice(S->device)); HIPCHK(hipStreamSynchronize(S->team->stream)); HIPCHK(hipDeviceSynchronize()); return NF_OK; }
void *nf_stream(nf_handle S) { return S ? (void *)S->team->stream : nullptr; }

extern "C" int nf_debug_xcd_buffer(void *h, double *out, int n, int coarse)
{
    nf_solver *S = (nf_solver *)h; if (!S || !S->team) return NF_ERR_ARG;
    nf_team *T = S->team;
    (void)coarse;
    if (!T->d_xpart) { for (int i = 0; i < n; ++i) out[i] = 0.0; return NF_OK; }
    HIPCHK(hipMemcpy(out, T->d_xpart, sizeof(double) * std::min(n, 512), hipMemcpyDeviceToHost));
    return NF_OK;
}
```

neutfem_amd/csrc/nf_kernels.h:

```cpp
#pragma once
#include <hip/hip_runtime.h>

#ifdef NF_STAMPS
#define NF_STAMP(buf, i) do { if (buf) (buf)[i] = (long long)__builtin_readcyclecounter(); } while (0)
#else
#define NF_STAMP(buf, i) do { } while (0)
#endif

#ifndef NF_SR_Z1_WAVES
#define NF_SR_Z1_WAVES 3
#endif
#ifndef NF_SR_Z2_WAVES
#define NF_SR_Z2_WAVES 4
#endif

namespace nf {

struct CgScalars {
    double rr, pAp, alpha, beta, rr_new, tol_sq, rhs_norm, tol;
    int done, its, maxit;
    int pend;
    int err;
    double rr2[2]; int its2[2];
};

struct HostPub { CgScalars cg; double out[8]; unsigned long long seq; };
__global__ void k_publish(const CgScalars *__restrict__ cg, const double *__restrict__ out, int nout, HostPub *hp, unsigned long long seq)
{
    if (threadIdx.x != 0 || blockIdx.x != 0) return;
    if (cg) hp->cg = *cg;
    for (int i = 0; i < nout && i < 8; ++i) hp->out[i] = out[i];
    __threadfence_system();
    __hip_atomic_store(&hp->seq, seq, __ATOMIC_RELEASE, __HIP_MEMORY_SCOPE_SYSTEM);
}

template <int CTRL, int ROW_MASK>
__device__ __forceinline__ double dpp_add(double v)
{
    const int lo = __builtin_amdgcn_update_dpp(0, __double2loint(v), CTRL, ROW_MASK, 0xF, true);
    const int hi = __builtin_amdgcn_update_dpp(0, __double2hiint(v), CTRL, ROW_MASK, 0xF, true);
    return v + __hiloint2double(hi, lo);
}
__device__ __forceinline__ double wave_sum(double v)
{
    v = dpp_add<0x111, 0xF>(v);
    v = dpp_add<0x112, 0xF>(v);
    v = dpp_add<0x114, 0xF>(v);
    v = dpp_add<0x118, 0xF>(v);
    v = dpp_add<0x142, 0xA>(v);
    v = dpp_add<0x143, 0xC>(v);
    return __hiloint2double(__builtin_amdgcn_readlane(__double2hiint(v), 63), __builtin_amdgcn_readlane(__double2loint(v), 63));
}

template <int CTRL, int ROW_MASK>
__device__ __forceinline__ double dpp_get(double v, double old)
{
    const int lo = __builtin_amdgcn_update_dpp(__double2loint(old), __double2loint(v), CTRL, ROW_MASK, 0xF, false);
    const int hi = __builtin_amdgcn_update_dpp(__double2hiint(old), __double2hiint(v), CTRL, ROW_MASK, 0xF, false);
    return __hiloint2double(hi, lo);
}
__device__ __forceinline__ double lane_above(double v) { return dpp_get<0x130, 0xF>(v, v); }
__device__ __forceinline__ double lane_below(double v) { return dpp_get<0x138, 0xF>(v, v); }
#define NF_SCAN_STEP(CTRL, D) if (LPL > D) { double Ap = dpp_get<CTRL, 0xF>(A, 1.0), Bp = dpp_get<CTRL, 0xF>(B, 0.0); \
                                             if (pos < D) { Ap = 1.0; Bp = 0.0; } B = A * Bp + B; A = A * Ap; }
__device__ __forceinline__ void scan_maps_up(double &A, double &B, int LPL, int lane)
{
    const int pos = lane & ((LPL < 16 ? LPL : 16) - 1);
    NF_SCAN_STEP(0x111, 1) NF_SCAN_STEP(0x112, 2) NF_SCAN_STEP(0x114, 4) NF_SCAN_STEP(0x118, 8)
    if (LPL > 16) { const double Ap = dpp_get<0x142, 0xA>(A, 1.0), Bp = dpp_get<0x142, 0xA>(B, 0.0); B = A * Bp + B; A = A * Ap; }
    if (LPL > 32) { const double Ap = dpp_get<0x143, 0xC>(A, 1.0), Bp = dpp_get<0x143, 0xC>(B, 0.0); B = A * Bp + B; A = A * Ap; }
}
#define NF_SCAN_STEP_DN(CTRL, D) if (LPL > D) { double Ap = dpp_get<CTRL, 0xF>(A, 1.0), Bp = dpp_get<CTRL, 0xF>(B, 0.0); \
                                                if (pos + D >= W) { Ap = 1.0; Bp = 0.0; } B = A * Bp + B; A = A * Ap; }
__device__ __forceinline__ void scan_maps_down(double &A, double &B, int LPL, int lane)
{
    const int W = LPL < 16 ? LPL : 16, pos = lane & (W - 1);
    NF_SCAN_STEP_DN(0x101, 1) NF_SCAN_STEP_DN(0x102, 2) NF_SCAN_STEP_DN(0x104, 4) NF_SCAN_STEP_DN(0x108, 8)
    if (LPL > 16) {
        const int src = (lane & ~31) + 16;
        double Ap = __shfl(A, src, 64), Bp = __shfl(B, src, 64);
        if (lane & 16) { Ap = 1.0; Bp = 0.0; }
        B = A * Bp + B; A = A * Ap;
    }
    if (LPL > 32) {
        double Ap = __shfl(A, 32, 64), Bp = __shfl(B, 32, 64);
        if (lane >= 32) { Ap = 1.0; Bp = 0.0; }
        B = A * Bp + B; A = A * Ap;
    }
}

__device__ __forceinline__ double strided_sum256(const double *__restrict__ p, int cnt)
{
    double s = 0.0;
    int i = threadIdx.x;
    if (threadIdx.x >= 256) return 0.0;
    for (; i + 7 * 256 < cnt; i += 8 * 256) {
        double v[8];
#pragma unroll
        for (int j = 0; j < 8; ++j) v[j] = p[i + j * 256];
#pragma unroll
        for (int j = 0; j < 8; ++j) s += v[j];
    }
    for (; i < cnt; i += 256) s += p[i];
    return s;
}
__device__ __forceinline__ double block_sum(double v, double *sred)
{
    v = wave_sum(v);
    const int lane = threadIdx.x & 63, w = threadIdx.x >> 6, nw = (blockDim.x + 63) >> 6;
    __syncthreads();
    if (lane == 0) sred[w] = v;
    __syncthreads();
    double s = 0.0;
    if (threadIdx.x == 0)
        for (int i = 0; i < nw; ++i) s += sred[i];
    return s;
}

__device__ __forceinline__ void block_sum3(double &a, double &b, double &c, double *sred)
{
    a = wave_sum(a); b = wave_sum(b); c = wave_sum(c);
    const int lane = threadIdx.x & 63, w = threadIdx.x >> 6, nw = (blockDim.x + 63) >> 6;
    __syncthreads();
    if (lane == 0) { sred[w] = a; sred[nw + w] = b; sred[2 * nw + w] = c; }
    __syncthreads();
    if (threadIdx.x == 0) {
        double sa = 0.0, sb = 0.0, sc = 0.0;
        for (int i = 0; i < nw; ++i) { sa += sred[i]; sb += sred[nw + i]; sc += sred[2 * nw + i]; }
        a = sa; b = sb; c = sc;
    }
}

struct PartSegs { int n; int off[16]; int cnt[16]; };
enum FinOp { FIN_RHS = 0, FIN_PAP = 1, FIN_RR = 2, FIN_SUM = 3 };

__device__ __forceinline__ int reduce_err(double total, double flag)
{
    return flag != 0.0 ? 2 : ((total - total) != 0.0 ? 1 : 0);
}
__device__ __forceinline__ void cg_logic(int op, const double *tot, int nq, CgScalars *cg, double *out, double tol, int maxit, double flag = 0.0)
{
    if (op == FIN_RHS) { cg->err = 0; }
    if (op != FIN_SUM) { const int e = reduce_err(tot[0], flag); if (e) { cg->err = e; cg->done = 1; if (op == FIN_RHS) { cg->rr = tot[0]; cg->its = 0; cg->pend = 0; } return; } }
    if (op == FIN_RHS) {
        cg->rr = tot[0];
        cg->rhs_norm = sqrt(tot[0]);
        cg->tol = tol;
        cg->tol_sq = tol * tol * cg->rhs_norm * cg->rhs_norm;
        cg->done = 0; cg->its = 0; cg->maxit = maxit; cg->pend = 0;
        cg->rr2[0] = tot[0]; cg->its2[0] = 0;
        if (maxit <= 0) cg->done = 1;
    } else if (op == FIN_PAP) {
        cg->pAp = tot[0];
        cg->pend = 0;
        if (fabs(tot[0]) < 1e-30) cg->done = 1;
        else cg->alpha = cg->rr / tot[0];
    } else if (op == FIN_RR) {
        cg->rr_new = tot[0];
        cg->its += 1;
        cg->pend = 1;
        if (tot[0] < cg->tol_sq) { cg->rr = tot[0]; cg->done = 1; }
        else {
            cg->beta = tot[0] / cg->rr;
            cg->rr = tot[0];
            if (cg->its >= cg->maxit) cg->done = 1;
        }
    } else {
        for (int q = 0; q < nq; ++q) out[q] = tot[q];
    }
}

__global__ __launch_bounds__(256) void k_finalize(int op, const double *__restrict__ partials, PartSegs segs, long stride,
                                                  int nq, CgScalars *__restrict__ cg, double *__restrict__ out,
                                                  double tol, int maxit, int reduce_only, double *__restrict__ red, const double *__restrict__ errsrc = nullptr)
{
    __shared__ double sred[4];
    if ((op == FIN_PAP || op == FIN_RR) && !reduce_only) { if (cg->done) return; }
    double tot[4] = { 0, 0, 0, 0 };
    for (int q = 0; q < nq; ++q) {
        double acc = 0.0;
        for (int sgi = 0; sgi < segs.n; ++sgi) {
            double s = strided_sum256(partials + q * stride + segs.off[sgi], segs.cnt[sgi]);
            s = block_sum(s, sred);
            acc += s;
        }
        tot[q] = acc;
    }
    if (threadIdx.x != 0) return;
    if (reduce_only) { for (int q = 0; q < nq; ++q) red[q] = tot[q]; if (errsrc) red[nq] = *errsrc; return; }
    cg_logic(op, tot, nq, cg, out, tol, maxit);
}
__global__ void k_cg_logic(int op, const double *__restrict__ red, int nq, CgScalars *__restrict__ cg, double *__restrict__ out,
                           double tol, int maxit, int with_flag)
{
    if (op == FIN_PAP || op == FIN_RR) { if (cg->done) return; }
// ... 592 lines not shown
        else for (int d = 1; d < LPL; d <<= 1) {
            const double Ap = __shfl_down(A, d, LPL), Bp = __shfl_down(B, d, LPL);
            if (li + d < LPL) { B = A * Bp + B; A = A * Ap; }
        }
        const double Ae = DPPS ? lane_above(A) : __shfl_down(A, 1, LPL), Be = DPPS ? lane_above(B) : __shfl_down(B, 1, LPL);
        double u = li == LPL - 1 ? ucarry : Ae * ucarry + Be;
        double uv[K];
#pragma unroll
        for (int j = K - 1; j >= 0; --j) { u = w[ch][j] - Lup[j] * u; uv[j] = u; }
        if (ch > 0) ucarry = __shfl(uv[0], 0, LPL);
        double ulo = DPPS ? lane_below(uv[K - 1]) : __shfl_up(uv[K - 1], 1, LPL);
        double wprev = 0.0;
        if (ch > 0) wprev = __shfl(w[ch > 0 ? ch - 1 : 0][K - 1], LPL - 1, LPL);
        if (li == 0) ulo = (ch == 0 ? z0 * d0 : wprev) - Ls[ch][0] * uv[0];
        double yv[NB + 1][K];
#pragma unroll
        for (int j = 0; j < K; ++j) {
            const double lo = j == 0 ? ulo : uv[j > 0 ? j - 1 : 0];
            yv[0][j] = (first ? yo[0][ch][j] * xm[0][ch][j] : yo[0][ch][j]) + ma.Ta * (uv[j] - lo);
            dot += xm[0][ch][j] * yv[0][j];
#pragma unroll
            for (int l = 0; l < NB; ++l) {
                const double v = ma.Gc[l] * xm[l + 1][ch][j] * ma.iM[l] * ic[ch][j] - (ma.eL[l] * lo + ma.eR[l] * uv[j]);
                yv[l + 1][j] = (first ? yo[l + 1][ch][j] * xm[l + 1][ch][j] : yo[l + 1][ch][j]) + ma.Ta * ma.Gc[l] * v;
                dot += xm[l + 1][ch][j] * yv[l + 1][j];
            }
        }
        const int c0 = (ch * LPL + li) * K;
#pragma unroll
        for (int q = 0; q <= NB; ++q) {
            if (VEC) { if (lv && c0 < nx) *reinterpret_cast<double2 *>(ma.y[q] + base + c0) = make_double2(yv[q][0], yv[q][K - 1]); }
            else {
#pragma unroll
                for (int j = 0; j < K; ++j) if (lv && c0 + j < nx) ma.y[q][base + c0 + j] = yv[q][j];
            }
        }
    }
    return dot;
}

template <int K, int NCH, bool VEC, int NB, bool NT = false, bool P2 = false, bool DICT = false>
__global__ __launch_bounds__(256) void k_schur_x(ModeArgs ma0, ModeTab mt, Geom G, const double *__restrict__ L, const double *__restrict__ DR,
                                                 const double *__restrict__ D0, int nx, int ny, long nlines, int lpl_log2,
                                                 int first, int last, double *__restrict__ partials,
                                                 const CgScalars *__restrict__ cg, CgFuse fz, CgLean lean, LineDict ld = LineDict())
{
    __shared__ double sred[4];
    if (cg && cg->done) return;
    const ModeArgs ma = select_mode(ma0, mt, blockIdx.y, NB + 1);
    const bool lean_on = lean.st && !lean.first;
    const bool fuse = fz.p != nullptr && (lean.st ? lean_on : cg->its > 0);
    const double alpha0 = fuse ? cg->alpha : 0.0, beta0 = (fuse && !lean.st) ? cg->beta : 0.0;
    LeanPre pre = { 0.0, 0.0, 0, 0 };
    if (lean_on) pre = lean_preload(lean);
    bool stopped = false;
    auto mid = [&](double &fa, double &fb) -> bool {
        (void)fa;
        if (lean_on) stopped = lean_rr_step(lean, pre, blockIdx.x == 0 && blockIdx.y == 0 && threadIdx.x == 0, sred, &fb);
        return stopped;
    };
    unsigned bx = blockIdx.x;
    if ((first & 2) && gridDim.x % 8 == 0) bx = (blockIdx.x % 8) * (gridDim.x / 8) + blockIdx.x / 8;
    const double dot = schur_x_task<K, NCH, VEC, NB, decltype(mid), false, NT, P2, DICT>(ma, G, L, DR, D0, nx, ny, nlines, lpl_log2, first & 1, (long)bx * 4 + (threadIdx.x >> 6),
                                                                               threadIdx.x & 63, true, fuse, alpha0, beta0, fz, mid, ld);
    if (stopped) return;
    if (last && partials) {
        const double s = block_sum(dot, sred);
        if (threadIdx.x == 0) partials[(long)blockIdx.y * gridDim.x + bx] = s;
    }
}

struct SlabArgs {
    int if_lo, if_hi, mode, xcd;
    int fold; const double *rlo, *rhi, *sinv_lo, *sinv_hi;
    int wsmin;
    int noacc; const double *yadd;
    const double *alo, *ahi, *ulo, *uhi;
    double *clo, *chi;
    double *jz;
    double *jzb;
    int nfa, ni, amode[9];
    Cg1 sr; double *sr_r; const double *sr_q; double *sr_part; long sr_stride;
};
enum : unsigned { SV_FUSE = 1, SV_NT = 2, SV_ZW = 4, SV_SR = 8, SV_DICT = 16, SV_ALL = 31 };
constexpr bool schur_s_legal(int SEG, int DIR, bool SLAB, int NB, unsigned V)
{
    const bool p0 = NB == 0, s8 = p0 && SEG == 8;
    const unsigned admits = (SLAB && p0 ? SV_FUSE : 0) | (s8 ? SV_NT : 0) | (!SLAB && p0 ? SV_ZW : 0) | (SLAB && s8 && DIR == 2 ? SV_SR : 0) | (!SLAB && (V & SV_NT) ? SV_DICT : 0);
    return (SEG == 4 || SEG == 8 || (p0 && (SEG == 16 || SEG == 32))) && (DIR == 2 || (DIR == 1 && !SLAB)) && NB >= 0 && NB <= 2 && !(V & ~admits);
}
template <int SEG, int DIR, bool SLAB, int NB, unsigned V = 0, class Mid = NoMid, bool XC = false>
__device__ __forceinline__ double schur_s_tile(const ModeArgs &ma, const Geom &G, const double *__restrict__ L, const double *__restrict__ DR,
                                               const double *__restrict__ D0, int n, long sl, long outer_stride, int nx, int TX, int NSEG,
                                               unsigned bx, unsigned by, unsigned bz, unsigned gy, int tid, bool act, double *sm,
                                               const SlabArgs &sa, const CgFuse &fz, bool fuse, bool fro, double f_alpha, double f_beta, bool acc,
                                               long long *stamp = nullptr, Mid mid = Mid(), double *extra = nullptr, const LineDict &ld = LineDict())
{
    constexpr bool FUSE = V & SV_FUSE, NT = V & SV_NT, ZW = V & SV_ZW, SR = V & SV_SR, DICT = V & SV_DICT;
    static_assert(SLAB || !(FUSE || SR), "fused update, single-reduction sums: slab passes (k_schur_s checks the rest: schur_s_legal)");
    const double *x = ma.x[0];
    double *__restrict__ y = ma.y[0];
    const int T = TX * NSEG;
    const bool wscan = NSEG >= (sa.wsmin > 0 ? sa.wsmin : 64) && NSEG <= 64 && (T & 63) == 0;
    const int NSP = wscan ? (NSEG | 1) : NSEG;
    const int TP = wscan ? TX * NSP : T;
    double *sA = sm, *sB = sm + TP, *sA2 = sm + 2 * TP, *sB2 = sm + 3 * TP, *sZ0 = sm + 4 * TP;
    act = act && tid < T;
    const int ixl = act ? tid % TX : 0, seg = act ? tid / TX : 0;
    const int si = wscan ? ixl * NSP + seg : seg * TX + ixl;
    const int ix = bx * TX + ixl;
    const bool valid = act && ix < nx;
    long base = (long)by * outer_stride + ix;
    const long lineid = (long)by * nx + ix;
    const long lm = SLAB ? (long)bz * ((long)nx * gy) + lineid : 0;
    const long roff = fro ? (long)(fz.r - fz.p) : 0;
    double x_before = 0.0, x_after = 0.0, a_lo = 0.0, a_hi = 0.0, u_lo = 0.0, u_hi = 0.0, xe_lo = 0.0, xe_hi = 0.0;
    long edge_lo = 0, edge_hi = 0;
    if (SLAB) {
        const int fs = sa.if_lo ? 1 : 0;
        const int nloc = n;
        n = nloc - fs - (sa.if_hi ? 1 : 0);
        edge_lo = base; edge_hi = base + (long)(nloc - 1) * sl;
        base += (long)fs * sl;
        if (valid) {
            if (sa.if_lo) {
                a_lo = sa.alo[lineid]; x_before = x[edge_lo];
                if (fuse) { if (seg == 0) fz.xsol[edge_lo] = fma(f_alpha, x_before, fz.xsol[edge_lo]);
                            x_before = fma(f_beta, x_before, (SR && FUSE) ? fma(-f_alpha, sa.sr_q[edge_lo], fz.r[edge_lo]) : fz.r[edge_lo]); }
                xe_lo = x_before;
                if (NB > 0) {
                    const double g1 = ma.Gc[0] * ma.x[1][edge_lo], g2 = NB > 1 ? ma.Gc[1] * ma.x[2][edge_lo] : 0.0;
                    xe_lo = x_before + ma.eL[0] * g1 + (NB > 1 ? ma.eL[1] * g2 : 0.0);
                    x_before = x_before - ma.eR[0] * g1 - (NB > 1 ? ma.eR[1] * g2 : 0.0);
                }
                if (sa.mode >= 2) { u_lo = sa.fold ? (sa.rlo[lm] + sa.clo[lm]) * sa.sinv_lo[lineid] : sa.ulo[lm]; x_before -= a_lo * u_lo; }
            }
            if (sa.if_hi) {
                a_hi = sa.ahi[lineid]; x_after = x[edge_hi];
                if (fuse) { if (seg == 0) fz.xsol[edge_hi] = fma(f_alpha, x_after, fz.xsol[edge_hi]);
                            x_after = fma(f_beta, x_after, (SR && FUSE) ? fma(-f_alpha, sa.sr_q[edge_hi], fz.r[edge_hi]) : fz.r[edge_hi]); }
                xe_hi = x_after;
                if (NB > 0) {
                    const double g1 = ma.Gc[0] * ma.x[1][edge_hi], g2 = NB > 1 ? ma.Gc[1] * ma.x[2][edge_hi] : 0.0;
                    xe_hi = x_after - ma.eR[0] * g1 - (NB > 1 ? ma.eR[1] * g2 : 0.0);
                    x_after = x_after + ma.eL[0] * g1 + (NB > 1 ? ma.eL[1] * g2 : 0.0);
                }
                if (sa.mode >= 2) { u_hi = sa.fold ? (sa.chi[lm] + sa.rhi[lm]) * sa.sinv_hi[lineid] : sa.uhi[lm]; x_after += a_hi * u_hi; }
            }
        }
    }
    const bool wr = !SLAB || sa.mode == 2;
    const int c0 = seg * SEG;
    double xv[SEG + 1], Lv[SEG + 1], Rv[SEG], yo[SEG];
    double x1[NB > 0 ? SEG : 1], x2[NB > 1 ? SEG : 1], icv[NB > 0 ? SEG : 1];
    double xLn = 0.0;
    if (SLAB && !FUSE) fuse = false;
    const bool fr = SLAB ? fuse : fro;
    constexpr bool O32 = NB > 0 && !SLAB;
    const unsigned ob8 = (unsigned)(base * 8), sl8 = (unsigned)(sl * 8);
    unsigned tb8 = 0;
    if (DICT) tb8 = valid ? (unsigned)ld.id[lineid] * (unsigned)ld.pitch * 8u : 0u;
#define NF_A8(c) (ob8 + (unsigned)(c) * sl8)
#define NF_T8(c) (tb8 + (unsigned)(c) * 8u)
    double rv[(SLAB && !FUSE) ? 1 : SEG + 1], sv[FUSE ? SEG : 1];
    double qv[(SR && FUSE) ? SEG + 1 : 1], rq_[(SR && !FUSE) ? SEG : 1];
    double srr = 0.0, sqq = 0.0, srq = 0.0;
    double r1[NB > 0 ? SEG + 1 : 1], r2[NB > 1 ? SEG + 1 : 1], v1a[NB > 0 ? SEG + 1 : 1], v2a[NB > 1 ? SEG + 1 : 1], Dv[NB > 0 ? SEG : 1];
#pragma unroll
    for (int i = 0; i <= SEG; ++i) {
        const int c = c0 + i; const bool ok = valid && c < n;
        const long a = base + (long)c * sl;
        if (O32) xv[i] = ok ? ldo<NT>(x, NF_A8(c)) : 0.0;
        else if (i < SEG || XC) xv[i] = ok ? ldg<NT>(x + a) : 0.0; else xv[i] = ok ? x[a] : 0.0;
        if (!SLAB || FUSE) rv[(SLAB && !FUSE) ? 0 : i] = (fr && ok) ? (SLAB ? fz.r[a] : (O32 ? ldo<NT>(x + roff, NF_A8(c)) : ldg<NT>(x + a + roff))) : 0.0;
        if (FUSE && i < SEG) sv[FUSE ? i : 0] = (fuse && ok) ? fz.xsol[a] : 0.0;
        if (SR && FUSE) qv[(SR && FUSE) ? i : 0] = (fuse && ok) ? sa.sr_q[a] : 0.0;
        if (DICT) { Lv[i] = ok ? ldo<false>(L, NF_T8(c)) : 0.0; if (i < SEG) Rv[i] = ok ? ldo<false>(DR, NF_T8(c)) : 0.0; }
        else if (O32) { Lv[i] = ok ? ldo<NT>(L, NF_A8(c)) : 0.0; if (i < SEG) Rv[i] = ok ? ldo<NT>(DR, NF_A8(c)) : 0.0; }
        else {
            if (i < SEG) Lv[i] = ok ? ldg<NT>(L + a) : 0.0; else Lv[i] = ok ? L[a] : 0.0;
            if (i < SEG) Rv[i] = ok ? ldg<NT>(DR + a) : 0.0;
        }
        if (NB > 0 && O32) {
            v1a[i] = ok ? ldo<XC>(ma.x[1], NF_A8(c)) : 0.0;
            if (NB > 1) v2a[NB > 1 ? i : 0] = ok ? ldo<XC>(ma.x[2], NF_A8(c)) : 0.0;
            r1[i] = (fro && ok) ? ldo<XC>(ma.x[1] + roff, NF_A8(c)) : 0.0;
            if (NB > 1) r2[NB > 1 ? i : 0] = (fro && ok) ? ldo<XC>(ma.x[2] + roff, NF_A8(c)) : 0.0;
            if (i < SEG) Dv[i] = ok ? ldo<false>(ma.D, NF_A8(c)) : 0.0;
        } else if (NB > 0) {
            v1a[i] = ok ? ldg<XC>(ma.x[1] + a) : 0.0;
            if (NB > 1) v2a[NB > 1 ? i : 0] = ok ? ldg<XC>(ma.x[2] + a) : 0.0;
            r1[i] = (!SLAB && fro && ok) ? ldg<XC>(ma.x[1] + a + roff) : 0.0;
            if (NB > 1) r2[NB > 1 ? i : 0] = (!SLAB && fro && ok) ? ldg<XC>(ma.x[2] + a + roff) : 0.0;
            if (i < SEG) Dv[i] = ok ? ma.D[a] : 0.0;
        }
    }
    double dinv_s = 0.0;
    if (DICT) { if (valid && c0 < n) dinv_s = c0 == 0 ? D0[lineid] : ldo<false>(DR, NF_T8(c0 - 1)); }
    else if (valid && c0 < n) dinv_s = c0 == 0 ? D0[lineid] : DR[base + (long)(c0 - 1) * sl];
    NF_STAMP(stamp, 3);
    if (mid(f_alpha, f_beta)) return 0.0;
#pragma unroll
    for (int i = 0; i <= SEG; ++i) {
        const int c = c0 + i; const bool ok = valid && c < n;
        if ((!SLAB || FUSE) && fr) {
            if (SR && FUSE) rv[(SLAB && !FUSE) ? 0 : i] = fma(-f_alpha, qv[(SR && FUSE) ? i : 0], rv[(SLAB && !FUSE) ? 0 : i]);
            if (FUSE && i < SEG) sv[FUSE ? i : 0] = fma(f_alpha, xv[i], sv[FUSE ? i : 0]);
            xv[i] = fma(f_beta, xv[i], rv[(SLAB && !FUSE) ? 0 : i]);
        }
        if (SR && FUSE && i < SEG) { const double rn = fr ? rv[(SLAB && !FUSE) ? 0 : i] : xv[i]; srr += ok ? rn * rn : 0.0; }
        if (SLAB && valid && c == n) xv[i] = x_after;
        if (NB > 0) {
            double v1 = v1a[i], v2 = NB > 1 ? v2a[NB > 1 ? i : 0] : 0.0;
            if (!SLAB && fro) { v1 = fma(f_beta, v1, r1[i]); if (NB > 1) v2 = fma(f_beta, v2, r2[NB > 1 ? i : 0]); }
            if (i < SEG) {
                x1[i] = v1; if (NB > 1) x2[NB > 1 ? i : 0] = v2;
                int cx = ix, cy = 0, cz = 0;
                if (DIR == 1) { cy = c; cz = by; } else { cy = by; cz = c + ((SLAB && sa.if_lo) ? 1 : 0); }
                icv[i] = ok ? Dv[i] / geom_factor(G, DIR, cx, cy, cz) : 0.0;
            } else {
                xLn = xv[i] + ma.eL[0] * ma.Gc[0] * v1 + (NB > 1 ? ma.eL[1] * ma.Gc[1] * v2 : 0.0);
                if (SLAB && valid && c == n) xLn = x_after;
            }
        }
    }
    if (FUSE && fuse) {
#pragma unroll
        for (int i = 0; i < SEG; ++i) if (valid && c0 + i < n) fz.xsol[base + (long)(c0 + i) * sl] = sv[FUSE ? i : 0];
    }
    double t[NB > 0 ? SEG : 1];
    double P = 1.0, lz = 0.0;
    double xL0 = xv[0];
    if (NB == 0) {
        (void)t;
    } else {
        double xLc[SEG + 1], xRc[SEG];
#pragma unroll
        for (int i = 0; i < SEG; ++i) {
            const double g1 = ma.Gc[0] * x1[i], g2 = NB > 1 ? ma.Gc[1] * x2[i] : 0.0;
            xLc[i] = xv[i] + ma.eL[0] * g1 + (NB > 1 ? ma.eL[1] * g2 : 0.0);
            xRc[i] = xv[i] - ma.eR[0] * g1 - (NB > 1 ? ma.eR[1] * g2 : 0.0);
        }
        xLc[SEG] = xLn; xL0 = xLc[0];
#pragma unroll
        for (int i = 0; i < SEG; ++i) t[i] = xRc[i] - xLc[i + 1];
    }
#pragma unroll
    for (int i = 0; i < SEG; ++i) { const double ti = NB == 0 ? xv[i] - xv[i + 1] : t[NB > 0 ? i : 0]; lz = ti - Lv[i] * lz; P = -Lv[i] * P; }
    NF_STAMP(stamp, 4);
    if (act) { sA[si] = P; sB[si] = lz; }
    if (act && seg == 0) sZ0[ixl] = x_before - xL0;
    __syncthreads();
    NF_STAMP(stamp, 5);
    if (wscan) {
        int W = 16; while (W < NSEG) W <<= 1;
        const int lane = tid & 63, cw = 64 / W, s_ = lane & (W - 1);
        if (tid < T)
            for (int c = (tid >> 6) * cw + lane / W; c < TX; c += (T >> 6) * cw) {
                double A = s_ < NSEG ? sA[c * NSP + s_] : 1.0, B = s_ < NSEG ? sB[c * NSP + s_] : 0.0;
                for (int d = 1; d < W; d <<= 1) {
                    const double Ap = __shfl_up(A, d, W), Bp = __shfl_up(B, d, W);
                    if (s_ >= d) { B = A * Bp + B; A = A * Ap; }
                }
                const double Ae = __shfl_up(A, 1, W), Be = __shfl_up(B, 1, W), z0 = sZ0[c];
                if (s_ < NSEG) sB[c * NSP + s_] = s_ == 0 ? z0 : Ae * z0 + Be;
            }
        __syncthreads();
    }
    if (SLAB && fuse && valid) {
#pragma unroll
        for (int i = 0; i < SEG; ++i) if (c0 + i < n) fz.p[base + (long)(c0 + i) * sl] = xv[i];
        if (seg == 0) { if (sa.if_lo) fz.p[edge_lo] = xe_lo; if (sa.if_hi) fz.p[edge_hi] = xe_hi; }
        if (SR && FUSE) {
#pragma unroll
            for (int i = 0; i < SEG; ++i) if (c0 + i < n) sa.sr_r[base + (long)(c0 + i) * sl] = rv[(SLAB && !FUSE) ? 0 : i];
            if (seg == 0) {
                if (sa.if_lo) { const double re = fma(-f_alpha, sa.sr_q[edge_lo], fz.r[edge_lo]); sa.sr_r[edge_lo] = re; srr += re * re; }
                if (sa.if_hi) { const double re = fma(-f_alpha, sa.sr_q[edge_hi], fz.r[edge_hi]); sa.sr_r[edge_hi] = re; srr += re * re; }
            }
        }
    }
    if (SR && FUSE && !fuse && valid && seg == 0) {
        if (sa.if_lo) { const double re = x[edge_lo]; srr += re * re; }
        if (sa.if_hi) { const double re = x[edge_hi]; srr += re * re; }
    }
    double z;
    if (wscan) z = sB[si];
    else { z = sZ0[ixl]; for (int s = 0; s < seg; ++s) z = sA[s * TX + ixl] * z + sB[s * TX + ixl]; }
    const double zin = z;
    double w[SEG];
    double zw = (ZW && c0 == 0) ? zin * (zin * dinv_s) : 0.0;
#pragma unroll
    for (int i = 0; i < SEG; ++i) { const double ti = NB == 0 ? xv[i] - xv[i + 1] : t[NB > 0 ? i : 0]; z = ti - Lv[i] * z; w[i] = z * Rv[i]; if (ZW) zw += z * w[i]; }
    if (ZW) asm volatile("" : "+v"(zw));
    double Q = 1.0, lu = 0.0;
#pragma unroll
    for (int i = SEG - 1; i >= 0; --i) { lu = w[i] - Lv[i + 1] * lu; Q = -Lv[i + 1] * Q; }
    if (act) { sA2[si] = Q; sB2[si] = lu; }
#pragma unroll
    for (int i = 0; i < SEG; ++i) {
        const int c = c0 + i; const bool ok = acc && valid && c < n && wr;
        yo[i] = ok ? (O32 ? ldo<NT>(y, NF_A8(c)) : ldg<NT>(y + base + (long)c * sl)) : 0.0;
        if (SLAB && NB == 0 && sa.yadd) yo[i] += ok ? sa.yadd[base + (long)c * sl] : 0.0;
    }
    double y1o[NB > 0 ? SEG : 1], y2o[NB > 1 ? SEG : 1];
    if (NB > 0) {
#pragma unroll
        for (int i = 0; i < SEG; ++i) {
            const bool okl = acc && valid && c0 + i < n && wr; const long a = base + (long)(c0 + i) * sl;
            y1o[i] = okl ? (O32 ? ldo<false>(ma.y[1], NF_A8(c0 + i)) : ma.y[1][a]) : 0.0;
            if (NB > 1) y2o[NB > 1 ? i : 0] = okl ? (O32 ? ldo<false>(ma.y[2], NF_A8(c0 + i)) : ma.y[2][a]) : 0.0;
        }
    }
    NF_STAMP(stamp, 6);
    __syncthreads();
    NF_STAMP(stamp, 7);
    if (SR && !FUSE) {
#pragma unroll
        for (int i = 0; i < SEG; ++i) rq_[(SR && !FUSE) ? i : 0] = (valid && c0 + i < n && wr) ? sa.sr_r[base + (long)(c0 + i) * sl] : 0.0;
    }
    double u = 0.0;
    if (wscan) {
        int W = 16; while (W < NSEG) W <<= 1;
        const int lane = tid & 63, cw = 64 / W, s_ = lane & (W - 1);
        if (tid < T)
            for (int c = (tid >> 6) * cw + lane / W; c < TX; c += (T >> 6) * cw) {
                double A = s_ < NSEG ? sA2[c * NSP + s_] : 1.0, B = s_ < NSEG ? sB2[c * NSP + s_] : 0.0;
                for (int d = 1; d < W; d <<= 1) {
                    const double Ap = __shfl_down(A, d, W), Bp = __shfl_down(B, d, W);
                    if (s_ + d < W) { B = A * Bp + B; A = A * Ap; }
                }
                const double Bn = __shfl_down(B, 1, W);
                if (s_ < NSEG) sA2[c * NSP + s_] = s_ == W - 1 ? 0.0 : Bn;
            }
        __syncthreads();
        if (act) u = sA2[si];
    } else if (act) for (int s = NSEG - 1; s > seg; --s) u = sA2[s * TX + ixl] * u + sB2[s * TX + ixl];
#pragma unroll
    for (int i = SEG - 1; i >= 0; --i) { u = w[i] - Lv[i + 1] * u; w[i] = u; }
    const double ulo = zin * dinv_s - Lv[0] * w[0];
    double dot = 0.0;
    if (wr) {
#pragma unroll
        for (int i = 0; i < SEG; ++i) {
            const double lo = i == 0 ? ulo : w[i > 0 ? i - 1 : 0];
            const bool in = valid && c0 + i < n;
            yo[i] = yo[i] + ma.Ta * (w[i] - lo); if (!ZW) dot += in ? xv[i] * yo[i] : 0.0;
            if (SR && !FUSE) { sqq += in ? yo[i] * yo[i] : 0.0; srq += in ? rq_[(SR && !FUSE) ? i : 0] * yo[i] : 0.0; }
            if (NB > 0) {
                const double v = ma.Gc[0] * x1[i] * ma.iM[0] * icv[i] - (ma.eL[0] * lo + ma.eR[0] * w[i]);
                y1o[i] = y1o[i] + ma.Ta * ma.Gc[0] * v; dot += in ? x1[i] * y1o[i] : 0.0;
            }
            if (NB > 1) {
                const double v = ma.Gc[1] * x2[NB > 1 ? i : 0] * ma.iM[1] * icv[i] - (ma.eL[1] * lo + ma.eR[1] * w[i]);
                y2o[NB > 1 ? i : 0] = y2o[NB > 1 ? i : 0] + ma.Ta * ma.Gc[1] * v; dot += in ? x2[NB > 1 ? i : 0] * y2o[NB > 1 ? i : 0] : 0.0;
            }
        }
#pragma unroll
        for (int i = 0; i < SEG; ++i) {
            const int c = c0 + i;
            if (valid && c < n) {
                const long a = base + (long)c * sl;
                if (O32) {
                    sto(y, NF_A8(c), yo[i]); sto(ma.y[1], NF_A8(c), y1o[i]);
                    if (NB > 1) sto(ma.y[2], NF_A8(c), y2o[NB > 1 ? i : 0]);
                } else {
                    y[a] = yo[i];
                    if (NB > 0) ma.y[1][a] = y1o[i];
                    if (NB > 1) ma.y[2][a] = y2o[NB > 1 ? i : 0];
                }
            }
        }
    }
    if (ZW) dot = ma.Ta * zw;
    if (SLAB && sa.mode == 3) {
        if (valid) {
            const long nxy = sl;
            int am = 0;
#pragma unroll
            for (int m = 0; m < 9; ++m) if ((unsigned)m == bz) am = sa.amode[m];
            const int fs = sa.if_lo ? 1 : 0, nfa = sa.nfa, kb = G.k, ni_ = sa.ni;
            double *const jz_ = sa.jz, *const jzb_ = sa.jzb;
            const double eL0 = ma.eL[0], eL1 = ma.eL[1], eR0 = ma.eR[0], eR1 = ma.eR[1], Gc0 = ma.Gc[0], Gc1 = ma.Gc[1], iM0 = ma.iM[0], iM1 = ma.iM[1];
            auto face = [=](long fpl) -> double & { return jz_[(fpl * nxy + lineid) * nfa + am]; };
            auto bubbles = [=](long cell, double lo, double hi, double xb1, double xb2, double ice) {
                for (int l = 0; l < kb; ++l) {
                    const double xb = l == 0 ? xb1 : xb2, Gl = l == 0 ? Gc0 : Gc1, iMl = l == 0 ? iM0 : iM1, eLl = l == 0 ? eL0 : eL1, eRl = l == 0 ? eR0 : eR1;
                    const double tb = l < NB ? Gl * xb * iMl * ice : 0.0;
                    jzb_[cell * ni_ + l + kb * am] = -(tb - (eLl * lo + eRl * hi));
                }
            };
#pragma unroll
            for (int i = 0; i < SEG; ++i) if (c0 + i < n) {
                face(fs + c0 + i + 1) = -w[i];
                if (kb > 0) bubbles((long)(fs + c0 + i) * nxy + lineid, i == 0 ? ulo : w[i > 0 ? i - 1 : 0], w[i], NB > 0 ? x1[NB > 0 ? i : 0] : 0.0, NB > 1 ? x2[NB > 1 ? i : 0] : 0.0,
                                    NB > 0 ? icv[NB > 0 ? i : 0] : 0.0);
            }
            if (seg == 0) {
                face(fs) = -ulo;
                if (sa.if_lo) {
                    const double us = sa.ulo[lm];
                    face(0) = -us;
                    if (kb > 0) bubbles(lineid, us, ulo, NB > 0 ? ma.x[NB > 0 ? 1 : 0][edge_lo] : 0.0, NB > 1 ? ma.x[NB > 1 ? 2 : 0][edge_lo] : 0.0,
                                        NB > 0 ? ma.D[edge_lo] / geom_factor(G, DIR, ix, (int)by, 0) : 0.0);
                }
            }
            if (sa.if_hi && c0 <= n - 1 && n - 1 < c0 + SEG) {
                double ulast = 0.0;
#pragma unroll
                for (int i = 0; i < SEG; ++i) if (c0 + i == n - 1) ulast = w[i];
                const double us = sa.uhi[lm];
                face(fs + n + 1) = -us;
                if (kb > 0) bubbles((long)(fs + n) * nxy + lineid, ulast, us, NB > 0 ? ma.x[NB > 0 ? 1 : 0][edge_hi] : 0.0, NB > 1 ? ma.x[NB > 1 ? 2 : 0][edge_hi] : 0.0,
                                    NB > 0 ? ma.D[edge_hi] / geom_factor(G, DIR, ix, (int)by, fs + n) : 0.0);
            }
        }
        return 0.0;
    }
    if (SLAB) {
        if (valid && seg == 0 && sa.if_lo) {
            const double a_lo = sa.alo[lineid];
            if (sa.mode == 1) sa.clo[lm] = -(NB == 0 ? x[edge_lo] : xe_lo) - a_lo * ulo;
            else {
                const double u_lo = sa.fold ? (sa.rlo[lm] + sa.clo[lm]) * sa.sinv_lo[lineid] : sa.ulo[lm];
                const double xe = x[edge_lo]; const double yv = (y[edge_lo] + ((NB == 0 && sa.yadd) ? sa.yadd[edge_lo] : 0.0)) + ma.Ta * (ulo - u_lo); y[edge_lo] = yv; dot += xe * yv;
                if (SR && !FUSE) { sqq += yv * yv; srq += sa.sr_r[edge_lo] * yv; }
                if (NB > 0) {
                    const double ice = ma.D[edge_lo] / geom_factor(G, DIR, ix, (int)by, 0);
#pragma unroll
                    for (int l = 0; l < NB; ++l) {
                        const double xb = ma.x[l + 1][edge_lo];
                        const double v = ma.Gc[l] * xb * ma.iM[l] * ice - (ma.eL[l] * u_lo + ma.eR[l] * ulo);
                        const double yb = ma.y[l + 1][edge_lo] + ma.Ta * ma.Gc[l] * v;
                        ma.y[l + 1][edge_lo] = yb; dot += xb * yb;
                    }
                }
            }
        }
        if (valid && sa.if_hi && c0 <= n - 1 && n - 1 < c0 + SEG) {
            double ulast = 0.0;
#pragma unroll
            for (int i = 0; i < SEG; ++i) if (c0 + i == n - 1) ulast = w[i];
            const double a_hi = sa.ahi[lineid];
            if (sa.mode == 1) sa.chi[lm] = (NB == 0 ? x[edge_hi] : xe_hi) - a_hi * ulast;
            else {
                const double u_hi = sa.fold ? (sa.chi[lm] + sa.rhi[lm]) * sa.sinv_hi[lineid] : sa.uhi[lm];
                const double xe = x[edge_hi]; const double yv = (y[edge_hi] + ((NB == 0 && sa.yadd) ? sa.yadd[edge_hi] : 0.0)) + ma.Ta * (u_hi - ulast); y[edge_hi] = yv; dot += xe * yv;
                if (SR && !FUSE) { sqq += yv * yv; srq += sa.sr_r[edge_hi] * yv; }
                if (NB > 0) {
                    const int fsz = sa.if_lo ? 1 : 0;
                    const double ice = ma.D[edge_hi] / geom_factor(G, DIR, ix, (int)by, fsz + n);
#pragma unroll
                    for (int l = 0; l < NB; ++l) {
                        const double xb = ma.x[l + 1][edge_hi];
                        const double v = ma.Gc[l] * xb * ma.iM[l] * ice - (ma.eL[l] * ulast + ma.eR[l] * u_hi);
                        const double yb = ma.y[l + 1][edge_hi] + ma.Ta * ma.Gc[l] * v;
                        ma.y[l + 1][edge_hi] = yb; dot += xb * yb;
                    }
                }
            }
        }
    }
    if (SR && FUSE) return srr;
    if (SR && extra) { extra[0] = sqq; extra[1] = srq; }
    return dot;
#undef NF_A8
#undef NF_T8
}

template <int SEG, int DIR, bool SLAB, int NB, unsigned V = 0>
__global__ __launch_bounds__(SLAB ? 512 : 1024, SLAB ? (NB > 0 ? 2 : ((V & SV_FUSE) ? ((V & SV_SR) ? NF_SR_Z1_WAVES : 3) : ((V & SV_SR) ? NF_SR_Z2_WAVES : 4))) : 1) void k_schur_s(ModeArgs ma0, ModeTab mt, Geom G, const double *__restrict__ L, const double *__restrict__ DR,
                          const double *__restrict__ D0, int n, long sl, long outer_stride, int nx, int TX, int NSEG,
                          int last, double *__restrict__ partials, const CgScalars *__restrict__ cg, SlabArgs sa, CgFuse fz, CgLean lean,
                          LineDict ld = LineDict())
{
    static_assert(schur_s_legal(SEG, DIR, SLAB, NB, V), "not a variant of k_schur_s");
    constexpr bool FUSE = V & SV_FUSE, SR = V & SV_SR;
    extern __shared__ double sm[];
    if (cg && cg->done) return;
    const ModeArgs ma = select_mode(ma0, mt, blockIdx.z, NB + 1);
    bool fuse = FUSE && sa.mode == 1 && fz.p != nullptr && (SR ? sa.sr.index > 0 : (lean.st ? !lean.first : cg->its > 0));
    double f_beta = fuse && !lean.st && !SR ? cg->beta : 0.0;
    if (SLAB && !SR && lean.st && !lean.first) {
        double *sred_l = sm + 4 * TX * (NSEG + 1) + TX;
        if (lean_rr_step(lean, blockIdx.x == 0 && blockIdx.y == 0 && blockIdx.z == 0 && threadIdx.x == 0, sred_l, &f_beta)) return;
    }
    double f_alpha = fuse && !SR ? cg->alpha : 0.0;
    if (SR && FUSE && fuse) { if (cg1_step(sa.sr, blockIdx.x == 0 && blockIdx.y == 0 && blockIdx.z == 0 && threadIdx.x == 0, &f_alpha, &f_beta)) return; }
    unsigned bx = blockIdx.x, by = blockIdx.y;
    if (sa.xcd) {
        const unsigned nblk = gridDim.x * gridDim.y, lin = blockIdx.y * gridDim.x + blockIdx.x;
        if (nblk % 8 == 0) { const unsigned nl = (lin % 8) * (nblk / 8) + lin / 8; bx = nl % gridDim.x; by = nl / gridDim.x; }
    }
    double extra[2] = { 0.0, 0.0 };
    const double dot = schur_s_tile<SEG, DIR, SLAB, NB, V>(ma, G, L, DR, D0, n, sl, outer_stride, nx, TX, NSEG, bx, by, blockIdx.z, gridDim.y,
                                                            (int)threadIdx.x, true, sm, sa, fz, fuse, false, f_alpha, f_beta, !(!SLAB && NB == 0 && sa.noacc),
                                                            nullptr, NoMid(), SR ? extra : nullptr, ld);
    if (SLAB && sa.mode == 3) return;
    double *sred = sm + 4 * TX * (NSEG + 1) + TX;
    const long pidx = ((long)blockIdx.z * gridDim.y + by) * gridDim.x + bx;
    if (SR && FUSE) {
        const double s = block_sum(dot, sred);
        if (threadIdx.x == 0) sa.sr_part[pidx] = s;
        return;
    }
    if (last && partials) {
        if (SR) {
            double s0 = dot, s1 = extra[0], s2 = extra[1];
            block_sum3(s0, s1, s2, sred);
            if (threadIdx.x == 0) { partials[pidx] = s0; partials[pidx + sa.sr_stride] = s1; partials[pidx + 2 * sa.sr_stride] = s2; }
        } else {
            const double s = block_sum(dot, sred);
            if (threadIdx.x == 0) partials[pidx] = s;
        }
    }
}

__global__ __launch_bounds__(256) void k_endpoint_w(double *__restrict__ p, double *__restrict__ r, const double *__restrict__ q, double *__restrict__ xsol,
                                                    const double *__restrict__ Wlo, const double *__restrict__ Whi, double *__restrict__ clo,
                                                    double *__restrict__ chi, int nx, int ny, int nz, int if_lo, int if_hi, int kcut, Cg1 sr,
                                                    const CgScalars *__restrict__ cg, double *__restrict__ rr_part)
{
    __shared__ double s_lo[4][64], s_hi[4][64], sred[4];
    if (cg && cg->done) return;
    double alpha = 0.0, beta = 0.0;
    const bool upd = sr.index > 0;
    if (upd && cg1_step(sr, blockIdx.x == 0 && blockIdx.y == 0 && threadIdx.x == 0, &alpha, &beta)) return;
    const int ixl = threadIdx.x & 63, seg = threadIdx.x >> 6;
    const int ix = blockIdx.x * 64 + ixl;
    const bool valid = ix < nx;
    const long nxy = (long)nx * ny, line = (long)blockIdx.y * nx + ix;
    const int per = (nz + 3) >> 2, k0 = seg * per, k1 = k0 + per < nz ? k0 + per : nz;
    double a_lo = 0.0, a_hi = 0.0, rr = 0.0;
    if (valid) {
#pragma unroll 4
        for (int k = k0; k < k1; ++k) {
            const long e = (long)k * nxy + line;
            double pv = p[e];
            if (upd) {
                const double rv = fma(-alpha, q[e], r[e]);
                xsol[e] = fma(alpha, pv, xsol[e]);
                pv = fma(beta, pv, rv);
                r[e] = rv; p[e] = pv; rr += rv * rv;
            } else rr += pv * pv;
            if (if_lo && k < kcut) a_lo = fma(Wlo[e], pv, a_lo);
            if (if_hi && k >= nz - kcut) a_hi = fma(Whi[e], pv, a_hi);
        }
    }
    s_lo[seg][ixl] = a_lo; s_hi[seg][ixl] = a_hi;
    __syncthreads();
    if (seg == 0 && valid) {
        if (if_lo) clo[line] = ((s_lo[0][ixl] + s_lo[1][ixl]) + s_lo[2][ixl]) + s_lo[3][ixl];
        if (if_hi) chi[line] = ((s_hi[0][ixl] + s_hi[1][ixl]) + s_hi[2][ixl]) + s_hi[3][ixl];
    }
    const double s = block_sum(rr, sred);
    if (threadIdx.x == 0) rr_part[(long)blockIdx.y * gridDim.x + blockIdx.x] = s;
}

constexpr bool schur_c_legal(int DIR, bool NT, bool DICT, int EARLY) { return (DIR == 1 || DIR == 2) && (!DICT || NT) && EARLY >= 0 && EARLY <= (DICT ? 2 : 0); }
template <int DIR, bool NT, bool DICT = false, int EARLY = 0>
__global__ __launch_bounds__(1024, 1) void k_schur_c(const double *__restrict__ x, double *__restrict__ y, double Ta,
                                                     const double *__restrict__ L, const double *__restrict__ DR, const double *__restrict__ D0,
// ... 2678 lines not shown
```

Baseline: 4.867 outer-iters/s.

## Add persistent staged Schur line kernel prefetching next tile into LDS

Adds an SV_STAGE variant of the segmented Schur line kernel for the dictionary/non-temporal path. It launches a persistent grid of about one block per CU, with each block looping over tiles. While the current tile is being computed, the next tile's x lines are loaded directly into LDS with global_load_lds, and raw s_barrier calls replace __syncthreads. The aim is to hide global load latency and cut launch and tail costs, at the price of extra LDS, fewer resident blocks, and fragile inline-asm ordering.

```diff
diff --git a/neutfem_amd/csrc/neutfem_hip.hip b/neutfem_amd/csrc/neutfem_hip.hip
--- a/neutfem_amd/csrc/neutfem_hip.hip
+++ b/neutfem_amd/csrc/neutfem_hip.hip
@@ -148,6 +148,7 @@
     int opt_line_dict = -1, line_dict_dirs = 7, line_dict_fp_bits = 128; long line_dict_max_bytes = 512L * 1024;
     int opt_s_long = -1, s_long_min = 256;
     int opt_c_early = -1;
+    int opt_s_stage = -1, opt_s_stage_grid = 0, ncu = 256;
     size_t lds_limit = 160 * 1024;
     int opt_fuse3 = 1; long fuse3_max_cells = 400000;
     int opt_sens_grid = RED_GRID;
@@ -435,6 +436,8 @@
         if (hipDeviceGetAttribute(&b, hipDeviceAttributeSharedMemPerBlockOptin, device) != hipSuccess) b = 0;
         (void)hipGetLastError();
         T->lds_limit = (size_t)std::max(std::max(a, b), 64 * 1024);
+        if (hipDeviceGetAttribute(&a, hipDeviceAttributeMultiprocessorCount, device) == hipSuccess && a > 0) T->ncu = a;
+        (void)hipGetLastError();
     }
     const char *cb = getenv("NEUTFEM_CG_BATCH"); T->cg_batch = cb ? atoi(cb) : 0;
     *out = S;
@@ -1254,6 +1257,22 @@
 static bool s_nt(const nf_solver *S, int zmode, int SEG) { return zmode != 3 && S->nb == 0 && SEG == 8 && nt_regime(S); }
 static bool s_dict(const nf_solver *S, int d, int zmode, int SEG) { return zmode == 0 && s_nt(S, zmode, SEG) && dict_dir(S, d); }
 static bool s_zw(const nf_solver *S, int zmode, bool zw_dot, bool want_dot) { return zmode == 0 && S->nb == 0 && zw_dot && want_dot; }
+static const int S_STAGE_AUTO_DIRS = 2;
+static size_t s_stage_bytes(int n, int TX) { const int rpp = 1024 / (8 * TX); return (size_t)((n + rpp - 1) / rpp) * 1024; }
+static unsigned s_stage_blocks(const nf_solver *S, const SegPlan &sp)
+{
+    const unsigned tiles = sp.grid.x * sp.grid.y, want = (unsigned)(S->team->opt_s_stage_grid > 0 ? S->team->opt_s_stage_grid : S->team->ncu);
+    return std::min(tiles, want);
+}
+static bool s_stage(const nf_solver *S, int d, int zmode, const SegPlan &sp, unsigned V)
+{
+    const nf_team *T = S->team;
+    if (zmode != 0 || T->opt_s_stage == 0 || !(V & SV_NT) || !(V & SV_DICT) || (V & ~(SV_NT | SV_DICT | SV_ZW))) return false;
+    if (sp.TX < 8 || sp.TX > 64 || (sp.TX & (sp.TX - 1)) || S->nx % sp.TX != 0) return false;
+    if (sp.lds + s_stage_bytes(d == 1 ? S->ny : S->nz, sp.TX) > T->lds_limit) return false;
+    if (T->opt_s_stage > 0) return true;
+    return ((S_STAGE_AUTO_DIRS >> (d - 1)) & 1) && sp.grid.x * sp.grid.y >= 2 * s_stage_blocks(S, sp);
+}
 static bool s_fold(const nf_team *T, int zmode) { return zmode == 2 && T->sep_sweeps == 0 && T->opt_sepfold; }
 static bool xcd_permutes(bool order, unsigned tiles) { return order && tiles % 8 == 0 && tiles > 8; }
 static SegPlan seg_plan(const nf_solver *S, int d, int zmode)
@@ -1346,9 +1365,9 @@
 struct SPass { int rc = NF_OK; bool chunked = false; ChunkPlan cp; SegPlan seg; unsigned V = 0; int xcd = 0, early = 0; bool fold = false, fuse = false; };
 static std::string variant_name(unsigned V)
 {
-    static const char *const bit[] = { "fuse", "nt", "zw", "sr", "dict" };
+    static const char *const bit[] = { "fuse", "nt", "zw", "sr", "dict", "stage" };
     std::string r;
-    for (int i = 0; i < 5; ++i) if (V >> i & 1) r += (r.empty() ? "" : "+") + std::string(bit[i]);
+    for (int i = 0; i < 6; ++i) if (V >> i & 1) r += (r.empty() ? "" : "+") + std::string(bit[i]);
     return r;
 }
 static SPass s_pass(const nf_solver *S, int d, int zmode, bool want_dot, bool zw_dot, bool fuse, bool cg1, bool chunks = true)
@@ -1368,6 +1387,7 @@
     const bool sr = cg1 && p0 && SEG == 8 && d == 2 && ((zmode == 1 && R.fuse) || (zmode == 2 && want_dot));
     R.V = (R.fuse && p0 ? SV_FUSE : 0) | (s_nt(S, zmode, SEG) ? SV_NT : 0) | (s_zw(S, zmode, zw_dot, want_dot) ? SV_ZW : 0)
         | (sr ? SV_SR : 0) | (s_dict(S, d, zmode, SEG) ? SV_DICT : 0);
+    if (s_stage(S, d, zmode, R.seg, R.V)) R.V |= SV_STAGE;
     R.xcd = s_xcd(S, d, zmode); R.fold = s_fold(S->team, zmode);
     return R;
 }
@@ -1435,17 +1455,32 @@
             sa.fold = 1; sa.rlo = S->d_rlo; sa.rhi = S->d_rhi; sa.sinv_lo = S->d_sinv_lo + g * nl; sa.sinv_hi = S->d_sinv_hi + g * nl;
         }
     }
+    if ((ps.V & SV_STAGE) && ((uintptr_t)ma.x[0] & 15)) ps.V &= ~SV_STAGE;
     int lg = 0; while ((4 << lg) < ps.seg.SEG) ++lg;
-    const unsigned key = (4 << lg) == ps.seg.SEG ? ((ps.V * 3 + (zmode != 0 ? 2u : d - 1u)) * 3 + (unsigned)S->nb) * 4 + (unsigned)lg : ~0u;
-    const bool hit = with_index<(SV_ALL + 1) * 3 * 3 * 4>(key, [&](auto i) {
-        constexpr unsigned I = decltype(i)::value, V = I / 36;
-        constexpr int SEG = 4 << (I & 3), NB = I / 4 % 3, DIR = I / 12 % 3 == 0 ? 1 : 2; constexpr bool SLAB = I / 12 % 3 == 2;
-        if constexpr (!schur_s_legal(SEG, DIR, SLAB, NB, V)) return false;
-        else hipLaunchKernelGGL((k_schur_s<SEG, DIR, SLAB, NB, V>), ps.seg.grid, ps.seg.block, ps.seg.lds, st, ma, mt, G, da.on ? da.L : L, da.on ? da.DR : DR, D0, n, sl, ostride, S->nx,
-                                ps.seg.TX, ps.seg.NSEG, last, partials, cg, sa, fz, lz, da.ld);
-        return true;
-    });
-    return hit ? NF_OK : fail(NF_ERR_ARG, "k_schur_s: no instantiation for SEG = %d (s_seg), direction %d, zmode %d, NB = %d, variant \"%s\"", ps.seg.SEG, d, zmode, S->nb, variant_name(ps.V).c_str());
+    for (;;) {
+        bool staged = true;
+        const unsigned key = (4 << lg) == ps.seg.SEG ? ((ps.V * 3 + (zmode != 0 ? 2u : d - 1u)) * 3 + (unsigned)S->nb) * 4 + (unsigned)lg : ~0u;
+        const bool hit = with_index<(SV_ALL + 1) * 3 * 3 * 4>(key, [&](auto i) {
+            constexpr unsigned I = decltype(i)::value, V = I / 36;
+            constexpr int SEG = 4 << (I & 3), NB = I / 4 % 3, DIR = I / 12 % 3 == 0 ? 1 : 2; constexpr bool SLAB = I / 12 % 3 == 2;
+            if constexpr (!schur_s_legal(SEG, DIR, SLAB, NB, V)) return false;
+            else if constexpr ((V & SV_STAGE) != 0) {
+                const size_t lds = ps.seg.lds + s_stage_bytes(n, ps.seg.TX);
+                const StageGrid sgr{ ps.seg.grid.x, ps.seg.grid.y };
+                staged = false;
+                if (lds_opt_in((const void *)k_schur_s<SEG, DIR, SLAB, NB, V>, lds)) {
+                    hipLaunchKernelGGL((k_schur_s<SEG, DIR, SLAB, NB, V>), dim3(s_stage_blocks(S, ps.seg), 1, ps.seg.grid.z), ps.seg.block, lds, st, ma, mt, G, da.on ? da.L : L, da.on ? da.DR : DR,
+                                       D0, n, sl, ostride, S->nx, ps.seg.TX, ps.seg.NSEG, last, partials, cg, sa, fz, lz, da.ld, sgr);
+                    staged = hipGetLastError() == hipSuccess;
+                }
+            }
+            else hipLaunchKernelGGL((k_schur_s<SEG, DIR, SLAB, NB, V>), ps.seg.grid, ps.seg.block, ps.seg.lds, st, ma, mt, G, da.on ? da.L : L, da.on ? da.DR : DR, D0, n, sl, ostride, S->nx,
+                                    ps.seg.TX, ps.seg.NSEG, last, partials, cg, sa, fz, lz, da.ld);
+            return true;
+        });
+        if (hit && (ps.V & SV_STAGE) && !staged) { ps.V &= ~SV_STAGE; continue; }
+        return hit ? NF_OK : fail(NF_ERR_ARG, "k_schur_s: no instantiation for SEG = %d (s_seg), direction %d, zmode %d, NB = %d, variant \"%s\"", ps.seg.SEG, d, zmode, S->nb, variant_name(ps.V).c_str());
+    }
 }
 
 static dim3 endpoint_w_grid(const nf_solver *S) { return dim3((unsigned)((S->nx + 63) / 64), (unsigned)S->ny); }
@@ -1776,7 +1811,7 @@
     return P;
 }
 
-struct PlanPass { const char *dir, *family; int mode, SEG, NCH, TX, NSEG; dim3 grid; unsigned block; bool nt, p2, zw, order; unsigned tiles; bool fold = false, dict = false; int early = 0; unsigned V = 0; };
+struct PlanPass { const char *dir, *family; int mode, SEG, NCH, TX, NSEG; dim3 grid; unsigned block; bool nt, p2, zw, order; unsigned tiles; bool fold = false, dict = false; int early = 0; unsigned V = 0, blocks = 0; };
 static void plan_emit(std::string &js, const PlanPass &p)
 {
     char tmp[416];
@@ -1785,6 +1820,7 @@
              p.SEG, p.NCH, p.TX, p.NSEG, p.grid.x, p.grid.y, p.grid.z, p.block, p.nt ? 1 : 0, p.p2 ? 1 : 0, p.zw ? 1 : 0, p.order ? 1 : 0, xcd_permutes(p.order, p.tiles) ? 1 : 0, p.fold ? 1 : 0, p.dict ? 1 : 0, p.early);
     js += tmp;
     if (!strcmp(p.family, "s")) js += ", \"variant\": \"" + variant_name(p.V) + "\"";
+    if (p.dir[0] != 'x') js += ", \"stage\": " + std::to_string((p.V & SV_STAGE) && !strcmp(p.family, "s") ? 1 : 0) + ", \"blocks\": " + std::to_string(p.blocks);
     js += "}";
 }
 static int plan_s(std::string &js, const nf_solver *S, int d, int zmode, bool want_dot, bool zw_dot, bool fuse, bool cg1)
@@ -1793,7 +1829,8 @@
     if (ps.rc != NF_OK) return ps.rc;
     const dim3 gr = ps.chunked ? c_grid(S, d, ps.cp) : ps.seg.grid;
     plan_emit(js, { d == 1 ? "y" : "z", ps.chunked ? "c" : "s", zmode, ps.chunked ? C_SEG : ps.seg.SEG, ps.chunked ? C_NCH : 1, ps.chunked ? ps.cp.TX : ps.seg.TX, ps.chunked ? ps.cp.NS : ps.seg.NSEG,
-                    gr, ps.chunked ? c_block(ps.cp) : ps.seg.block.x, (ps.V & SV_NT) != 0, false, (ps.V & SV_ZW) != 0, ps.xcd != 0, gr.x * gr.y, ps.fold, (ps.V & SV_DICT) != 0, ps.early, ps.V });
+                    gr, ps.chunked ? c_block(ps.cp) : ps.seg.block.x, (ps.V & SV_NT) != 0, false, (ps.V & SV_ZW) != 0, ps.xcd != 0, gr.x * gr.y, ps.fold, (ps.V & SV_DICT) != 0, ps.early, ps.V,
+                    !ps.chunked && (ps.V & SV_STAGE) ? s_stage_blocks(S, ps.seg) * gr.z : gr.x * gr.y * gr.z });
     return NF_OK;
 }
 int nf_apply_plan(nf_handle S, int in_cg, char *json_buf, size_t len)
@@ -2301,7 +2338,7 @@
     C->opt_line_dict = T->opt_line_dict; C->line_dict_dirs = T->line_dict_dirs; C->line_dict_fp_bits = T->line_dict_fp_bits; C->line_dict_max_bytes = T->line_dict_max_bytes;
     C->opt_nt_loads = T->opt_nt_loads; C->nt_min_cells = T->nt_min_cells; C->opt_s_long = T->opt_s_long; C->opt_s_long_dirs = T->opt_s_long_dirs;
     C->s_long_min = T->s_long_min; C->s_long_min_y = T->s_long_min_y; C->opt_s_seg = T->opt_s_seg; C->opt_s_tx = T->opt_s_tx;
-    C->opt_wsmin = T->opt_wsmin; C->opt_c_early = T->opt_c_early; C->opt_x_p2 = T->opt_x_p2; C->opt_split_dot = T->opt_split_dot; C->opt_xcd = T->opt_xcd;
+    C->opt_wsmin = T->opt_wsmin; C->opt_c_early = T->opt_c_early; C->opt_s_stage = T->opt_s_stage; C->opt_s_stage_grid = T->opt_s_stage_grid; C->opt_x_p2 = T->opt_x_p2; C->opt_split_dot = T->opt_split_dot; C->opt_xcd = T->opt_xcd;
     C->opt_xy_overlap = T->opt_xy_overlap; C->xy_overlap_max_cells = T->xy_overlap_max_cells; C->opt_vec_reduce = T->opt_vec_reduce;
     C->opt_pub = T->opt_pub; C->opt_sens_grid = T->opt_sens_grid; C->prof_every = T->prof_every;
     if (dict_moved) { (void)hipSetDevice(C->device); for (auto *X : C->slabs) line_dict_drop(X); }
@@ -4811,6 +4848,8 @@
     else if (!strcmp(key, "s_long_min_y")) T->s_long_min_y = (int)std::max(1L, std::min(1000000L, value));
     else if (!strcmp(key, "s_long_min")) T->s_long_min = (int)std::max(1L, std::min(1000000L, value));
     else if (!strcmp(key, "c_early")) T->opt_c_early = value < 0 ? -1 : (int)std::min(2L, value);
+    else if (!strcmp(key, "s_stage")) T->opt_s_stage = value < 0 ? -1 : (value > 0 ? 1 : 0);
+    else if (!strcmp(key, "s_stage_grid")) T->opt_s_stage_grid = (int)std::max(0L, std::min(1L << 20, value));
     else if (!strcmp(key, "line_dict") || !strcmp(key, "line_dict_dirs") || !strcmp(key, "line_dict_max_bytes") || !strcmp(key, "line_dict_fp_bits")) {
         if (!strcmp(key, "line_dict")) T->opt_line_dict = value < 0 ? -1 : (value > 0 ? 1 : 0);
         else if (!strcmp(key, "line_dict_dirs")) T->line_dict_dirs = (int)(value & 7);
diff --git a/neutfem_amd/csrc/nf_kernels.h b/neutfem_amd/csrc/nf_kernels.h
--- a/neutfem_amd/csrc/nf_kernels.h
+++ b/neutfem_amd/csrc/nf_kernels.h
@@ -12,6 +12,9 @@
 #endif
 #ifndef NF_SR_Z2_WAVES
 #define NF_SR_Z2_WAVES 4
+#endif
+#ifndef NF_STAGE_PLACE
+#define NF_STAGE_PLACE 1
 #endif
 
 namespace nf {
@@ -104,13 +107,19 @@
     for (; i < cnt; i += 256) s += p[i];
     return s;
 }
+template <bool RAW> __device__ __forceinline__ void block_bar()
+{
+    if constexpr (RAW) { asm volatile("s_waitcnt lgkmcnt(0)" ::: "memory"); __builtin_amdgcn_s_barrier(); asm volatile("" ::: "memory"); }
+    else __syncthreads();
+}
+template <bool RAW = false>
 __device__ __forceinline__ double block_sum(double v, double *sred)
 {
     v = wave_sum(v);
     const int lane = threadIdx.x & 63, w = threadIdx.x >> 6, nw = (blockDim.x + 63) >> 6;
-    __syncthreads();
+    block_bar<RAW>();
     if (lane == 0) sred[w] = v;
-    __syncthreads();
+    block_bar<RAW>();
     double s = 0.0;
     if (threadIdx.x == 0)
         for (int i = 0; i < nw; ++i) s += sred[i];
@@ -869,21 +878,42 @@
     int nfa, ni, amode[9];
     Cg1 sr; double *sr_r; const double *sr_q; double *sr_part; long sr_stride;
 };
-enum : unsigned { SV_FUSE = 1, SV_NT = 2, SV_ZW = 4, SV_SR = 8, SV_DICT = 16, SV_ALL = 31 };
+enum : unsigned { SV_FUSE = 1, SV_NT = 2, SV_ZW = 4, SV_SR = 8, SV_DICT = 16, SV_STAGE = 32, SV_ALL = 63 };
 constexpr bool schur_s_legal(int SEG, int DIR, bool SLAB, int NB, unsigned V)
 {
     const bool p0 = NB == 0, s8 = p0 && SEG == 8;
-    const unsigned admits = (SLAB && p0 ? SV_FUSE : 0) | (s8 ? SV_NT : 0) | (!SLAB && p0 ? SV_ZW : 0) | (SLAB && s8 && DIR == 2 ? SV_SR : 0) | (!SLAB && (V & SV_NT) ? SV_DICT : 0);
+    const unsigned admits = (SLAB && p0 ? SV_FUSE : 0) | (s8 ? SV_NT : 0) | (!SLAB && p0 ? SV_ZW : 0) | (SLAB && s8 && DIR == 2 ? SV_SR : 0) | (!SLAB && (V & SV_NT) ? SV_DICT : 0)
+                            | (!SLAB && s8 && (V & SV_NT) && (V & SV_DICT) ? SV_STAGE : 0);
     return (SEG == 4 || SEG == 8 || (p0 && (SEG == 16 || SEG == 32))) && (DIR == 2 || (DIR == 1 && !SLAB)) && NB >= 0 && NB <= 2 && !(V & ~admits);
+}
+struct StageCtx {
+    const double *buf = nullptr, *next = nullptr;
+    const int *next_id = nullptr;
+    int id = 0;
+};
+template <bool NT>
+__device__ __forceinline__ void stage_issue(const double *buf, const double *src, int n, long sl, int TX)
+{
+    typedef __attribute__((address_space(1))) const void *gptr_t;
+    typedef __attribute__((address_space(3))) void *lptr_t;
+    const int lane = threadIdx.x & 63, w = __builtin_amdgcn_readfirstlane(threadIdx.x >> 6), nw = blockDim.x >> 6;
+    const int lpr = TX >> 1, rpp = 64 / lpr;
+    const int rl = lane / lpr, cl = lane % lpr;
+    const char *dst = reinterpret_cast<const char *>(buf);
+    for (int p = w, np = (n + rpp - 1) / rpp; p < np; p += nw) {
+        const int r = p * rpp + rl;
+        if (r < n) __builtin_amdgcn_global_load_lds((gptr_t)(src + (long)r * sl + 2 * cl), (lptr_t)(dst + p * 1024), 16, 0, NT ? 2 : 0);
+    }
 }
 template <int SEG, int DIR, bool SLAB, int NB, unsigned V = 0, class Mid = NoMid, bool XC = false>
 __device__ __forceinline__ double schur_s_tile(const ModeArgs &ma, const Geom &G, const double *__restrict__ L, const double *__restrict__ DR,
                                                const double *__restrict__ D0, int n, long sl, long outer_stride, int nx, int TX, int NSEG,
                                                unsigned bx, unsigned by, unsigned bz, unsigned gy, int tid, bool act, double *sm,
                                                const SlabArgs &sa, const CgFuse &fz, bool fuse, bool fro, double f_alpha, double f_beta, bool acc,
-                                               long long *stamp = nullptr, Mid mid = Mid(), double *extra = nullptr, const LineDict &ld = LineDict())
-{
-    constexpr bool FUSE = V & SV_FUSE, NT = V & SV_NT, ZW = V & SV_ZW, SR = V & SV_SR, DICT = V & SV_DICT;
+                                               long long *stamp = nullptr, Mid mid = Mid(), double *extra = nullptr, const LineDict &ld = LineDict(),
+                                               StageCtx *sg = nullptr)
+{
+    constexpr bool FUSE = V & SV_FUSE, NT = V & SV_NT, ZW = V & SV_ZW, SR = V & SV_SR, DICT = V & SV_DICT, STAGE = V & SV_STAGE;
     static_assert(SLAB || !(FUSE || SR), "fused update, single-reduction sums: slab passes (k_schur_s checks the rest: schur_s_legal)");
     const double *x = ma.x[0];
     double *__restrict__ y = ma.y[0];
@@ -946,7 +976,8 @@
     constexpr bool O32 = NB > 0 && !SLAB;
     const unsigned ob8 = (unsigned)(base * 8), sl8 = (unsigned)(sl * 8);
     unsigned tb8 = 0;
-    if (DICT) tb8 = valid ? (unsigned)ld.id[lineid] * (unsigned)ld.pitch * 8u : 0u;
+    if constexpr (STAGE) tb8 = valid ? (unsigned)sg->id * (unsigned)ld.pitch * 8u : 0u;
+    else if (DICT) tb8 = valid ? (unsigned)ld.id[lineid] * (unsigned)ld.pitch * 8u : 0u;
 #define NF_A8(c) (ob8 + (unsigned)(c) * sl8)
 #define NF_T8(c) (tb8 + (unsigned)(c) * 8u)
     double rv[(SLAB && !FUSE) ? 1 : SEG + 1], sv[FUSE ? SEG : 1];
@@ -957,7 +988,8 @@
     for (int i = 0; i <= SEG; ++i) {
         const int c = c0 + i; const bool ok = valid && c < n;
         const long a = base + (long)c * sl;
-        if (O32) xv[i] = ok ? ldo<NT>(x, NF_A8(c)) : 0.0;
+        if constexpr (STAGE) { const double v = sg->buf[(c < n ? c : n - 1) * TX + ixl]; xv[i] = ok ? v : 0.0; }
+        else if (O32) xv[i] = ok ? ldo<NT>(x, NF_A8(c)) : 0.0;
         else if (i < SEG || XC) xv[i] = ok ? ldg<NT>(x + a) : 0.0; else xv[i] = ok ? x[a] : 0.0;
         if (!SLAB || FUSE) rv[(SLAB && !FUSE) ? 0 : i] = (fr && ok) ? (SLAB ? fz.r[a] : (O32 ? ldo<NT>(x + roff, NF_A8(c)) : ldg<NT>(x + a + roff))) : 0.0;
         if (FUSE && i < SEG) sv[FUSE ? i : 0] = (fuse && ok) ? fz.xsol[a] : 0.0;
@@ -1037,8 +1069,14 @@
     NF_STAMP(stamp, 4);
     if (act) { sA[si] = P; sB[si] = lz; }
     if (act && seg == 0) sZ0[ixl] = x_before - xL0;
-    __syncthreads();
+    if constexpr (STAGE) {
+#pragma unroll
+        for (int i = 0; i < SEG; ++i) asm volatile("" :: "v"(Rv[i]));
+        asm volatile("" :: "v"(dinv_s));
+    }
+    block_bar<STAGE>();
     NF_STAMP(stamp, 5);
+    if constexpr (STAGE && NF_STAGE_PLACE == 0) { if (sg->next) { stage_issue<NT>(sg->buf, sg->next, n, sl, TX); sg->id = sg->next_id[ixl]; } }
     if (wscan) {
         int W = 16; while (W < NSEG) W <<= 1;
         const int lane = tid & 63, cw = 64 / W, s_ = lane & (W - 1);
@@ -1052,7 +1090,7 @@
                 const double Ae = __shfl_up(A, 1, W), Be = __shfl_up(B, 1, W), z0 = sZ0[c];
                 if (s_ < NSEG) sB[c * NSP + s_] = s_ == 0 ? z0 : Ae * z0 + Be;
             }
-        __syncthreads();
+        block_bar<STAGE>();
     }
     if (SLAB && fuse && valid) {
 #pragma unroll
@@ -1099,8 +1137,9 @@
             if (NB > 1) y2o[NB > 1 ? i : 0] = okl ? (O32 ? ldo<false>(ma.y[2], NF_A8(c0 + i)) : ma.y[2][a]) : 0.0;
         }
     }
+    if constexpr (STAGE && NF_STAGE_PLACE == 1) { if (sg->next) { stage_issue<NT>(sg->buf, sg->next, n, sl, TX); sg->id = sg->next_id[ixl]; } }
     NF_STAMP(stamp, 6);
-    __syncthreads();
+    block_bar<STAGE>();
     NF_STAMP(stamp, 7);
     if (SR && !FUSE) {
 #pragma unroll
@@ -1120,7 +1159,7 @@
                 const double Bn = __shfl_down(B, 1, W);
                 if (s_ < NSEG) sA2[c * NSP + s_] = s_ == W - 1 ? 0.0 : Bn;
             }
-        __syncthreads();
+        block_bar<STAGE>();
         if (act) u = sA2[si];
     } else if (act) for (int s = NSEG - 1; s > seg; --s) u = sA2[s * TX + ixl] * u + sB2[s * TX + ixl];
 #pragma unroll
@@ -1142,6 +1181,12 @@
                 const double v = ma.Gc[1] * x2[NB > 1 ? i : 0] * ma.iM[1] * icv[i] - (ma.eL[1] * lo + ma.eR[1] * w[i]);
                 y2o[NB > 1 ? i : 0] = y2o[NB > 1 ? i : 0] + ma.Ta * ma.Gc[1] * v; dot += in ? x2[NB > 1 ? i : 0] * y2o[NB > 1 ? i : 0] : 0.0;
             }
+        }
+        if constexpr (STAGE) {
+#pragma unroll
+            for (int i = 0; i < SEG; ++i) asm volatile("" : "+v"(yo[i]));
+            asm volatile("" : "+v"(sg->id));
+            asm volatile("s_waitcnt vmcnt(0)" ::: "memory");
         }
 #pragma unroll
         for (int i = 0; i < SEG; ++i) {
@@ -1255,16 +1300,50 @@
 #undef NF_T8
 }
 
+struct StageGrid { unsigned gx = 0, gy = 0; };
 template <int SEG, int DIR, bool SLAB, int NB, unsigned V = 0>
 __global__ __launch_bounds__(SLAB ? 512 : 1024, SLAB ? (NB > 0 ? 2 : ((V & SV_FUSE) ? ((V & SV_SR) ? NF_SR_Z1_WAVES : 3) : ((V & SV_SR) ? NF_SR_Z2_WAVES : 4))) : 1) void k_schur_s(ModeArgs ma0, ModeTab mt, Geom G, const double *__restrict__ L, const double *__restrict__ DR,
                           const double *__restrict__ D0, int n, long sl, long outer_stride, int nx, int TX, int NSEG,
                           int last, double *__restrict__ partials, const CgScalars *__restrict__ cg, SlabArgs sa, CgFuse fz, CgLean lean,
-                          LineDict ld = LineDict())
+                          LineDict ld = LineDict(), StageGrid sgr = StageGrid())
 {
     static_assert(schur_s_legal(SEG, DIR, SLAB, NB, V), "not a variant of k_schur_s");
     constexpr bool FUSE = V & SV_FUSE, SR = V & SV_SR;
     extern __shared__ double sm[];
     if (cg && cg->done) return;
+    if constexpr (V & SV_STAGE) {
+        const ModeArgs ma = select_mode(ma0, mt, blockIdx.z, NB + 1);
+        double *sred = sm + 4 * TX * (NSEG + 1) + TX;
+        const double *buf = sred + 32;
+        const unsigned gx = sgr.gx, gy = sgr.gy, tiles = gx * gy;
+        const bool remap = sa.xcd && tiles % 8 == 0;
+        auto origin = [&](unsigned t, unsigned &bx, unsigned &by) {
+            const unsigned nl = remap ? (t % 8) * (tiles / 8) + t / 8 : t;
+            bx = nl % gx; by = nl / gx;
+        };
+        auto tile_x = [&](unsigned t) { unsigned bx, by; origin(t, bx, by); return ma.x[0] + ((long)by * outer_stride + (long)bx * TX); };
+        auto tile_id = [&](unsigned t) { unsigned bx, by; origin(t, bx, by); return ld.id + ((long)by * nx + (long)bx * TX); };
+        const int ixl0 = (int)threadIdx.x < TX * NSEG ? (int)threadIdx.x % TX : 0;
+        unsigned t = blockIdx.x;
+        StageCtx sg; sg.buf = buf;
+        if (t < tiles) { stage_issue<(V & SV_NT) != 0>(buf, tile_x(t), n, sl, TX); sg.id = tile_id(t)[ixl0]; }
+        asm volatile("s_waitcnt vmcnt(0)" ::: "memory");
+        asm volatile("" : "+v"(sg.id));
+        for (; t < tiles; t += gridDim.x) {
+            unsigned bx, by; origin(t, bx, by);
+            const bool more = t + gridDim.x < tiles;
+            sg.next = more ? tile_x(t + gridDim.x) : nullptr; sg.next_id = more ? tile_id(t + gridDim.x) : nullptr;
+            block_bar<true>();
+            const double dot = schur_s_tile<SEG, DIR, SLAB, NB, V>(ma, G, L, DR, D0, n, sl, outer_stride, nx, TX, NSEG, bx, by, blockIdx.z, gy,
+                                                                    (int)threadIdx.x, true, sm, sa, fz, false, false, 0.0, 0.0, !sa.noacc,
+                                                                    nullptr, NoMid(), nullptr, ld, &sg);
+            if (last && partials) {
+                const double s = block_sum<true>(dot, sred);
+                if (threadIdx.x == 0) partials[((long)blockIdx.z * gy + by) * gx + bx] = s;
+            }
+        }
+        return;
+    }
     const ModeArgs ma = select_mode(ma0, mt, blockIdx.z, NB + 1);
     bool fuse = FUSE && sa.mode == 1 && fz.p != nullptr && (SR ? sa.sr.index > 0 : (lean.st ? !lean.first : cg->its > 0));
     double f_beta = fuse && !lean.st && !SR ? cg->beta : 0.0;
```

After: 5.011 outer-iters/s (median of 6 runs). 1.03x the previous value.
